# servos/SLAM

Measured on AMD Instinct MI355X. Metric: registered_scan_points_per_s, higher is better.
Workload: dtype f64 pose / f32 distance / int32 counts

## Files before the change

### slam_amd/csrc/grid.hip

```cpp
#include <algorithm>
#include <cmath>
#include <cstdlib>
#include <cstring>
#include <memory>
#include <vector>

#include "device_mem.hpp"
#include "grid_cell.hpp"

using namespace slam;

namespace {

struct GridView {
    int      sx, sy;
    int      ox, oy;
    double   res;
    double   max_range;
    double   pose_x, pose_y;
    int      rolling;
    int32_t *hits;
    int32_t *misses;
    unsigned long long *updates;
    int     *dirty;
    const int32_t *acc_hits, *acc_misses;
};

__device__ inline int storage_index(const GridView &g, int x, int y)
{
    int ix = x + g.ox, iy = y + g.oy;
    if (ix >= g.sx) ix -= g.sx;
    if (iy >= g.sy) iy -= g.sy;
    return ix + g.sx * iy;
}

__device__ inline bool point_cell(const GridView &g, float px, float py, int *cx, int *cy)
{
    return point_cell_of(g.sx, g.sy, g.res, g.max_range, g.pose_x, g.pose_y, g.rolling, px, py, cx, cy);
}

constexpr int kUpdateSlots = 1024;

__device__ inline void mark_dirty_rows(int *dirty, int row_lo, int row_hi )
{
    int lo = row_hi >= 0 ? row_lo : 0x7fffffff, nhi = row_hi >= 0 ? -row_hi : 0x7fffffff;
    for (int off = 32; off > 0; off >>= 1) {
        lo = min(lo, __shfl_xor(lo, off));
        nhi = min(nhi, __shfl_xor(nhi, off));
    }
    if ((threadIdx.x & 63) == 0 && lo != 0x7fffffff) {
        if (lo < __hip_atomic_load(&dirty[0], __ATOMIC_RELAXED, __HIP_MEMORY_SCOPE_AGENT)) atomicMin(&dirty[0], lo);
        if (nhi < __hip_atomic_load(&dirty[1], __ATOMIC_RELAXED, __HIP_MEMORY_SCOPE_AGENT)) atomicMin(&dirty[1], nhi);
    }
}

__device__ inline void block_add_updates(unsigned long long *slots, unsigned n)
{
    for (int off = 32; off > 0; off >>= 1) n += __shfl_xor((int)n, off);
    if ((threadIdx.x & 63) == 0 && n) {
        const unsigned wave = (blockIdx.x * (blockDim.x >> 6) + (threadIdx.x >> 6)) + blockIdx.y * 7919u;
        atomicAdd(&slots[wave & (kUpdateSlots - 1)], (unsigned long long)n);
    }
}

constexpr int kEndpointsPerBlock = 1024;

__global__ __launch_bounds__(256) void endpoints_kernel(GridView g, const float *obs, int n_obs,
                                                        const float *gnd, int n_gnd, int stride)
{
    __shared__ int      s_lo[4], s_nhi[4];
    __shared__ unsigned s_cnt[4];
    const int lane = threadIdx.x & 63, wave = threadIdx.x >> 6;
    int       lo = 0x7fffffff, nhi = 0x7fffffff;
    unsigned  cnt = 0;
#pragma unroll
    for (int k = 0; k < kEndpointsPerBlock / 256; ++k) {
        const int i = blockIdx.x * kEndpointsPerBlock + k * 256 + (int)threadIdx.x;
        bool      did = false;
        int       key = -1;
        if (i < n_obs + n_gnd) {
            const bool   is_obs = i < n_obs;
            const float *p = is_obs ? obs + (size_t)i * stride : gnd + (size_t)(i - n_obs) * stride;
            int cx, cy;
            if (point_cell(g, p[0], p[1], &cx, &cy)) {
                const int s = storage_index(g, cx, cy), row = s / g.sx;
                did = true;
                key = (is_obs ? 0 : g.sx * g.sy) + s;
                lo = min(lo, row);
                nhi = min(nhi, -row);
                ++cnt;
            }
        }
        const int                prev = __shfl_up(key, 1);
        const bool               head = did && (lane == 0 || prev != key);
        const unsigned long long heads = __ballot(head || !did);
        if (head) {
            const unsigned long long after = lane == 63 ? 0ull : heads >> (lane + 1);
            const int                len = after ? __builtin_ctzll(after) + 1 : 64 - lane;
            atomicAdd(&g.hits[key], len);
        }
    }
    for (int off = 32; off > 0; off >>= 1) {
        lo = min(lo, __shfl_xor(lo, off));
        nhi = min(nhi, __shfl_xor(nhi, off));
        cnt += (unsigned)__shfl_xor((int)cnt, off);
    }
    if (lane == 0) s_lo[wave] = lo, s_nhi[wave] = nhi, s_cnt[wave] = cnt;
    __syncthreads();
    if (threadIdx.x == 0) {
        lo = min(min(s_lo[0], s_lo[1]), min(s_lo[2], s_lo[3]));
        nhi = min(min(s_nhi[0], s_nhi[1]), min(s_nhi[2], s_nhi[3]));
        cnt = s_cnt[0] + s_cnt[1] + s_cnt[2] + s_cnt[3];
        if (lo != 0x7fffffff) {
            if (lo < __hip_atomic_load(&g.dirty[0], __ATOMIC_RELAXED, __HIP_MEMORY_SCOPE_AGENT)) atomicMin(&g.dirty[0], lo);
            if (nhi < __hip_atomic_load(&g.dirty[1], __ATOMIC_RELAXED, __HIP_MEMORY_SCOPE_AGENT)) atomicMin(&g.dirty[1], nhi);
        }
        if (cnt) atomicAdd(&g.updates[(blockIdx.x * 7u + blockIdx.y * 7919u) & (kUpdateSlots - 1)], (unsigned long long)cnt);
    }
}

struct Beam {
    short x0, y0, x1, y1;
};

constexpr int kTile = 128;
#ifndef SLAM_WALK_UNROLL
#define SLAM_WALK_UNROLL 4
#endif
constexpr int kWalkUnroll = SLAM_WALK_UNROLL;
#ifndef SLAM_WALK_STAGGER
#define SLAM_WALK_STAGGER 8
#endif
constexpr int kWalkStagger = SLAM_WALK_STAGGER;
constexpr int kTileStride = kTile + 1;
constexpr int kTileThreads = 1024;
constexpr int kChunk = 1024;
constexpr int kBlock = 64;

__device__ inline Beam make_beam(const GridView &g, float ox, float oy, float ex, float ey)
{
    Beam b;
    b.x0 = -1;
    b.y0 = b.x1 = b.y1 = 0;
    int x1, y1, x0, y0;
    if (!point_cell(g, ex, ey, &x1, &y1)) return b;
    if (!cell_coord(ox, g.res, g.sx / 2, &x0)) return b;
    if (!cell_coord(oy, g.res, g.sy / 2, &y0)) return b;
    if (x0 < 0 || y0 < 0 || x0 >= g.sx || y0 >= g.sy) return b;
    b.x0 = (short)x0;
    b.y0 = (short)y0;
    b.x1 = (short)x1;
    b.y1 = (short)y1;
    return b;
}

__device__ inline void store_beam_and_box(const Beam &b, bool in_range, int i, Beam *beams, int4 *block_box)
{
    if (in_range) beams[i] = b;
    const bool ok = in_range && b.x0 >= 0;
    int lo_x = ok ? min((int)b.x0, (int)b.x1) : 0x7fffffff, lo_y = ok ? min((int)b.y0, (int)b.y1) : 0x7fffffff;
    int hi_x = ok ? max((int)b.x0, (int)b.x1) : -1, hi_y = ok ? max((int)b.y0, (int)b.y1) : -1;
    for (int off = 32; off > 0; off >>= 1) {
        lo_x = min(lo_x, __shfl_xor(lo_x, off));
        lo_y = min(lo_y, __shfl_xor(lo_y, off));
        hi_x = max(hi_x, __shfl_xor(hi_x, off));
        hi_y = max(hi_y, __shfl_xor(hi_y, off));
    }
    if ((threadIdx.x & 63) == 0) block_box[i >> 6] = make_int4(lo_x, lo_y, hi_x, hi_y);
}

__global__ __launch_bounds__(kChunk) void beams_from_rays_kernel(GridView g, const float2 *origin,
                                                                 const float2 *end, int n, Beam *beams,
                                                                 int4 *block_box)
{
    const int  i = blockIdx.x * kChunk + threadIdx.x;
    const bool in = i < n;
    Beam       b;
    b.x0 = -1;
    b.y0 = b.x1 = b.y1 = 0;
    if (in) {
        const float2 o = origin[i], e = end[i];
        b = make_beam(g, o.x, o.y, e.x, e.y);
    }
    store_beam_and_box(b, in, i, beams, block_box);
}

__global__ __launch_bounds__(kChunk) void beams_from_scans_kernel(GridView g, const double2 *pts,
                                                                  const int *scan_off, int n_scans,
                                                                  const double *R, const double *t, int n,
                                                                  Beam *beams, int4 *block_box)
{
    const int  i = blockIdx.x * kChunk + threadIdx.x;
    const bool in = i < n;
    Beam       b;
    b.x0 = -1;
    b.y0 = b.x1 = b.y1 = 0;
    if (in) {
        int lo = (int)(((long long)i * n_scans) / max(n, 1));
        lo = min(max(lo, 0), n_scans - 1);
        int steps = 0;
        while (steps < 4 && scan_off[lo] > i) --lo, ++steps;
        while (steps < 4 && lo + 1 < n_scans && scan_off[lo + 1] <= i) ++lo, ++steps;
        if (scan_off[lo] > i || (lo + 1 < n_scans && scan_off[lo + 1] <= i)) {
            lo = 0;
            int hi = n_scans - 1;
            while (lo < hi) {
                const int mid = (lo + hi + 1) >> 1;
                if (scan_off[mid] <= i)
                    lo = mid;
                else
                    hi = mid - 1;
            }
        }
        const double *Rs = R + 4 * (size_t)lo, *ts = t + 2 * (size_t)lo;
        const double2 P = pts[i];
        const double cx = g.rolling ? g.pose_x : 0.0, cy = g.rolling ? g.pose_y : 0.0;
        const double gx = __dadd_rn(__dadd_rn(__dmul_rn(Rs[0], P.x), __dmul_rn(Rs[1], P.y)), ts[0]);
        const double gy = __dadd_rn(__dadd_rn(__dmul_rn(Rs[2], P.x), __dmul_rn(Rs[3], P.y)), ts[1]);
        const float  ex = (float)(g.rolling ? __dsub_rn(gx, cx) : gx), ey = (float)(g.rolling ? __dsub_rn(gy, cy) : gy);
        const float  ox = (float)(g.rolling ? __dsub_rn(ts[0], cx) : ts[0]);
        const float  oy = (float)(g.rolling ? __dsub_rn(ts[1], cy) : ts[1]);
        b = make_beam(g, ox, oy, ex, ey);
    }
    store_beam_and_box(b, in, i, beams, block_box);
}

__global__ __launch_bounds__(256) void raycast_global_kernel(GridView g, const Beam *beams, int n)
{
    const int i = blockIdx.x * 256 + threadIdx.x;
    unsigned  did = 0;
    int       rlo = 0, rhi = -1;
    if (i < n) {
        const Beam b = beams[i];
        if (b.x0 >= 0) {
            const int dx = abs(b.x1 - b.x0), dy = abs(b.y1 - b.y0);
            const int sx = b.x1 > b.x0 ? 1 : -1, sy = b.y1 > b.y0 ? 1 : -1;
            int x = b.x0, y = b.y0;
            if (dx >= dy) {
                int e = dx;
                for (int k = 0; k < dx; ++k) {
                    atomicAdd(&g.misses[storage_index(g, x, y)], 1);
                    x += sx;
                    e += 2 * dy;
                    if (e >= 2 * dx) {
                        y += sy;
                        e -= 2 * dx;
                    }
                }
                did = dx + 1;
            } else {
                int e = dy;
                for (int k = 0; k < dy; ++k) {
                    atomicAdd(&g.misses[storage_index(g, x, y)], 1);
                    y += sy;
                    e += 2 * dx;
                    if (e >= 2 * dy) {
                        x += sx;
                        e -= 2 * dy;
                    }
                }
                did = dy + 1;
            }
            atomicAdd(&g.hits[storage_index(g, b.x1, b.y1)], 1);
            const int ra = storage_index(g, 0, b.y0) / g.sx, rb = storage_index(g, 0, b.y1) / g.sx;
            const bool wraps = (ra <= rb) != (b.y0 <= b.y1);
            rlo = wraps ? 0 : min(ra, rb);
            rhi = wraps ? g.sy - 1 : max(ra, rb);
        }
    }
    mark_dirty_rows(g.dirty, rlo, rhi);
    block_add_updates(g.updates, did);
}


__device__ inline bool box_overlaps_tile(const int4 cb, int tx0, int ty0, int tx1, int ty1)
{
    return cb.z >= tx0 && cb.x <= tx1 && cb.w >= ty0 && cb.y <= ty1;
}

constexpr int kMaxLdsTiles = 2048;

template <int FILL>
__global__ __launch_bounds__(256) void tile_items_kernel(const int4 *block_box, int n_blocks, int tiles_x,
                                                         int n_tiles, int sx, int sy, int *cnt,
                                                         const int *item_off, int *items)
{
    const int t = (blockIdx.x * 256 + threadIdx.x) >> 6, lane = threadIdx.x & 63;
    if (t >= n_tiles) return;
    const int tx0 = (t % tiles_x) * kTile, ty0 = (t / tiles_x) * kTile;
    const int tx1 = min(tx0 + kTile, sx) - 1, ty1 = min(ty0 + kTile, sy) - 1;
    int       c = 0;
    const int base_out = FILL == 1 ? item_off[t] : 0;
    for (int base = 0; base < n_blocks; base += 256) {
        int4 cb[4];
#pragma unroll
        for (int j = 0; j < 4; ++j) {
            const int ch = base + 64 * j + lane;
            cb[j] = ch < n_blocks ? block_box[ch] : make_int4(0, 0, -1, -1);
        }
#pragma unroll
        for (int j = 0; j < 4; ++j) {
            const bool               ov = box_overlaps_tile(cb[j], tx0, ty0, tx1, ty1);
            const unsigned long long m = __ballot(ov);
            if (FILL && ov) items[base_out + c + __popcll(m & ((1ull << lane) - 1ull))] = base + 64 * j + lane;
            c += __popcll(m);
        }
    }
    if (FILL != 1 && lane == 0) cnt[t] = c;
}

__global__ __launch_bounds__(1024) void tile_items_wg_kernel(const int4 *block_box, int n_blocks, int tiles_x, int sx,
                                                             int sy, int *cnt, int *items, int *cursor)
{
    __shared__ int s_cnt[4][16], s_base;
    const int t = blockIdx.x, tid = threadIdx.x, lane = tid & 63, wave = tid >> 6;
    if (tid == 0) {
        s_base = 0;
        cursor[t] = 0;
        if (t == 0) cursor[gridDim.x] = 0;
    }
    const int tx0 = (t % tiles_x) * kTile, ty0 = (t / tiles_x) * kTile;
    const int tx1 = min(tx0 + kTile, sx) - 1, ty1 = min(ty0 + kTile, sy) - 1;
    const int base_out = t * n_blocks;
    for (int base = 0; base < n_blocks; base += 4096) {
        int4 cb[4];
#pragma unroll
        for (int j = 0; j < 4; ++j) {
            const int ch = base + 1024 * j + tid;
            cb[j] = ch < n_blocks ? block_box[ch] : make_int4(0, 0, -1, -1);
        }
        unsigned long long m[4];
#pragma unroll
        for (int j = 0; j < 4; ++j) {
            m[j] = __ballot(box_overlaps_tile(cb[j], tx0, ty0, tx1, ty1));
            if (lane == 0) s_cnt[j][wave] = __popcll(m[j]);
        }
        __syncthreads();
        int total = 0;
#pragma unroll
        for (int j = 0; j < 4; ++j)
            for (int w = 0; w < 16; ++w) {
                const int c = s_cnt[j][w];
                total += c;
            }
        int run = s_base;
#pragma unroll
        for (int j = 0; j < 4; ++j) {
            int mine = run;
            for (int w = 0; w < 16; ++w) {
                const int c = s_cnt[j][w];
                mine += w < wave ? c : 0;
                run += c;
            }
            if ((m[j] >> lane) & 1ull)
                items[base_out + mine + __popcll(m[j] & ((1ull << lane) - 1ull))] = base + 1024 * j + tid;
        }
        __syncthreads();
        if (tid == 0) s_base += total;
    }
    __syncthreads();
    if (tid == 0) cnt[t] = s_base;
}

__global__ __launch_bounds__(1024) void tile_scan_kernel(const int *cnt, int n_tiles, int *item_off, int *cursor)
{
    __shared__ int carry;
    __shared__ int wsum[16];
    const int tid = threadIdx.x;
    if (tid == 0) carry = 0;
    __syncthreads();
    for (int base = 0; base < n_tiles; base += 1024) {
        const int i = base + tid;
        const int v0 = i < n_tiles ? cnt[i] : 0;
        int       x0 = v0;
        for (int off = 1; off < 64; off <<= 1) {
            const int y0 = __shfl_up(x0, off);
            if ((tid & 63) >= off) x0 += y0;
        }
        if ((tid & 63) == 63) wsum[tid >> 6] = x0;
        __syncthreads();
        int w0 = 0;
        for (int w = 0; w < (tid >> 6); ++w) w0 += wsum[w];
        const int in0 = carry + w0 + x0;
        if (i < n_tiles) {
            item_off[i] = in0 - v0;
            cursor[i] = 0;
        }
        __syncthreads();
        if (tid == 1023) carry = in0;
        __syncthreads();
    }
    if (tid == 0) {
        item_off[n_tiles] = carry;
        cursor[n_tiles] = 0;
    }
}

__device__ inline int floor_div_small(int num, int den, float rden)
{
    const float qf = (float)num * rden;
    if (qf >= 65536.0f) return 65536;
    int       q = (int)qf;
    const int r = (int)((unsigned)num - (unsigned)__mul24(q, den));
    q += (r >= den) - (r < 0);
    return q;
}

constexpr int kChunkMin = 8;
constexpr int kChunkDefault = 16;
constexpr int kMaxAccBlocks = 1023;

template <bool MERGE>
__global__ __launch_bounds__(kTileThreads, 8) void raycast_tiled_kernel(GridView g, const Beam *beams, int n,
                                                                        const int *items, const int *item_off,
                                                                        int n_tiles, int *cursor, int tiles_x, int chunk,
                                                                        int ablate_arg, const int *cnt, int item_stride)
{
#ifdef SLAM_MEASURE
    const int ablate = ablate_arg;
#else
    constexpr int ablate = 0;
    (void)ablate_arg;
#endif
    __shared__ __attribute__((aligned(16))) unsigned tile[kTile * kTileStride];
    __shared__ int s_ticket, s_done, s_end;
    __shared__ unsigned long long s_desc[kMaxAccBlocks / kChunkMin];
    __shared__ int s_off[kMaxLdsTiles + 1], s_wsum[kTileThreads / 64], s_carry;
    __shared__ unsigned long long s_best[kTileThreads / 64];

    const int tid = threadIdx.x, lane = tid & 63;
    const bool in_lds = item_off == nullptr;
    if (in_lds) {
        if (tid == 0) s_carry = 0;
        __syncthreads();
        for (int base = 0; base < n_tiles; base += kTileThreads) {
            const int i = base + tid;
            const int v = i < n_tiles ? cnt[i] : 0;
            int       x = v;
            for (int off = 1; off < 64; off <<= 1) {
                const int y = __shfl_up(x, off);
                if (lane >= off) x += y;
            }
            if (lane == 63) s_wsum[tid >> 6] = x;
            __syncthreads();
            int w = 0;
            for (int k = 0; k < (tid >> 6); ++k) w += s_wsum[k];
            const int incl = s_carry + w + x;
            if (i < n_tiles) s_off[i] = incl - v;
            __syncthreads();
            if (tid == kTileThreads - 1) s_carry = incl;
            __syncthreads();
        }
        if (tid == 0) s_off[n_tiles] = s_carry;
        __syncthreads();
    }
    const auto list_start = [&](int t) { return in_lds ? s_off[t] : item_off[t]; };
    const int  total = list_start(n_tiles);
    unsigned   did = 0;
    int        d_lo = 0x7fffffff, d_hi = -1;
    if (total <= 0 || (ablate & 8)) {
        mark_dirty_rows(g.dirty, d_lo, d_hi);
        block_add_updates(g.updates, did);
        return;
    }
    int cur;
    {
        const int pos = (int)(((long long)blockIdx.x * total) / gridDim.x);
        int       lo = 0, hi = n_tiles - 1;
        while (lo < hi) {
            const int mid = (lo + hi + 1) >> 1;
            if (list_start(mid) <= pos)
                lo = mid;
            else
                hi = mid - 1;
        }
        cur = lo;
    }
    for (int i = tid * 4; i < kTile * kTileStride; i += kTileThreads * 4)
        *reinterpret_cast<uint4 *>(&tile[i]) = make_uint4(0u, 0u, 0u, 0u);

    const auto flush = [&](int t) {
        const int tx0 = (t % tiles_x) * kTile, ty0 = (t / tiles_x) * kTile;
        for (int i = (ablate & 2) ? kTile * kTile : tid; i < kTile * kTile; i += kTileThreads) {
            const int      lx = i & (kTile - 1), ly = i / kTile;
            const unsigned v = tile[ly * kTileStride + lx];
            if (!v) continue;
            tile[ly * kTileStride + lx] = 0u;
            const int s = storage_index(g, tx0 + lx, ty0 + ly);
            if (ablate & 128) {
                atomicAdd(reinterpret_cast<unsigned long long *>(g.hits) + s, ((unsigned long long)(v >> 16) << 32) | (v & 0xffffu));
            } else {
                if (v & 0xffffu) atomicAdd(&g.misses[s], (int)(v & 0xffffu));
                if (v >> 16) atomicAdd(&g.hits[s], (int)(v >> 16));
            }
            int row = ty0 + ly + g.oy;
            row -= row >= g.sy ? g.sy : 0;
            d_lo = min(d_lo, row);
            d_hi = max(d_hi, row);
        }
        if (tid == 0) atomicAdd(&cursor[n_tiles], 1);
    };

    const int  kMaxChunks = kMaxAccBlocks / chunk;
    const auto publish = [&](int c, int base, int np) {
        __hip_atomic_store(&s_desc[c], (1ull << 48) | ((unsigned long long)(unsigned)np << 32) | (unsigned)base, __ATOMIC_RELAXED,
                           __HIP_MEMORY_SCOPE_WORKGROUP);
        if (np < chunk) {
            atomicMin(&s_end, np > 0 ? c + 1 : c);
            s_done = 1;
        }
    };
    for (;;) {
        __syncthreads();
        for (int c = tid; c < kMaxChunks; c += kTileThreads) s_desc[c] = 0ull;
        if (tid == 0) {
            s_ticket = 0;
            s_done = 0;
            s_end = kMaxChunks;
        }
        __syncthreads();
        const int t = cur;
        if (tid == 0) {
            const int have_t = cnt[t];
            const int k = atomicAdd(&cursor[t], 2 * chunk);
            const int np0 = max(0, min(chunk, have_t - k));
            publish(0, k, np0);
            if (np0 == chunk) publish(1, k + chunk, max(0, min(chunk, have_t - k - chunk)));
        }
        const int tile_base = in_lds ? t * item_stride : item_off[t];
        const int tx0 = (t % tiles_x) * kTile, ty0 = (t / tiles_x) * kTile;
        const int tx1 = min(tx0 + kTile, g.sx) - 1, ty1 = min(ty0 + kTile, g.sy) - 1;

        int  fetch_c = -1, fetch_k = 0;
        auto settle = [&]() {
            if (fetch_c >= 0 && lane == 0) publish(fetch_c, fetch_k, max(0, min(chunk, cnt[t] - fetch_k)));
            fetch_c = -1;
        };
        auto wait_desc = [&](int c) -> unsigned long long {
            for (;;) {
                if (c >= __hip_atomic_load(&s_end, __ATOMIC_RELAXED, __HIP_MEMORY_SCOPE_WORKGROUP)) return 0ull;
                const unsigned long long d = __hip_atomic_load(&s_desc[c], __ATOMIC_RELAXED, __HIP_MEMORY_SCOPE_WORKGROUP);
                if (d != 0ull) return d;
                if (fetch_c >= 0)
                    settle();
                else
                    __builtin_amdgcn_s_sleep(1);
            }
        };
        auto grab = [&](int2 *raw) -> bool {
            int T = 0;
            if (lane == 0) T = atomicAdd(&s_ticket, 1);
            T = __builtin_amdgcn_readfirstlane(T);
            const int c = T / chunk, idx = T - c * chunk;
            if (c >= kMaxChunks) return false;
            const unsigned long long d = wait_desc(c);
            const int np = (int)((d >> 32) & 0xffffu), base = (int)(unsigned)(d & 0xffffffffull);
            if (idx >= np) return false;
            if (idx == 0 && np == chunk && c + 2 < kMaxChunks) {
                const unsigned long long d1 = wait_desc(c + 1);
                if ((int)((d1 >> 32) & 0xffffu) == chunk) {
                    settle();
                    if (lane == 0) fetch_k = atomicAdd(&cursor[t], chunk);
                    fetch_c = c + 2;
                }
            }
            const int bi = items[tile_base + base + idx] * kBlock + lane;
            *raw = bi < n ? *reinterpret_cast<const int2 *>(&beams[bi]) : make_int2(-1, 0);
            return true;
        };
        int2 raw = make_int2(-1, 0), raw_next = make_int2(-1, 0);
        bool have = grab(&raw);
        while (have) {
            const bool have_next = grab(&raw_next);

            int rem = 0, a = 0, e = 0, dv2 = 0, den = 1, step_u = 0, step_v = 0, to_end = 0;
            const int x0 = (short)(raw.x & 0xffff), y0 = raw.x >> 16;
            const int x1 = (short)(raw.y & 0xffff), y1 = raw.y >> 16;
            const bool maybe = x0 >= 0 && max(x0, x1) >= tx0 && min(x0, x1) <= tx1 && max(y0, y1) >= ty0 &&
                               min(y0, y1) <= ty1;
            if (__any(maybe) && !(ablate & 16)) {
                const int dx = abs(x1 - x0), dy = abs(y1 - y0);
                const bool xm = dx >= dy;
                const int  u0 = xm ? x0 : y0, v0 = xm ? y0 : x0, u1 = xm ? x1 : y1, v1 = xm ? y1 : x1;
                const int  du = xm ? dx : dy, dv = xm ? dy : dx;
                const int  tu0 = xm ? tx0 : ty0, tu1 = xm ? tx1 : ty1;
                const int  tv0 = xm ? ty0 : tx0, tv1 = xm ? ty1 : tx1;
                const bool up = u1 > u0, vp = v1 > v0;
                int        i_lo = max(0, up ? tu0 - u0 : u0 - tu1);
                int        i_hi = min(du, up ? tu1 - u0 : u0 - tu0);
                den = max(2 * du, 1);
                dv2 = 2 * dv;
                const float rden = __builtin_amdgcn_rcpf((float)den);
                const int k_lo = vp ? tv0 - v0 : v0 - tv1;
                const int k_hi = min(vp ? tv1 - v0 : v0 - tv0, dv);
                bool      enters = maybe && k_hi >= 0 && k_lo <= dv;
                if (enters && dv > 0 && !(ablate & 32)) {
                    const float rdv2 = __builtin_amdgcn_rcpf((float)dv2);
                    if (k_lo > 0) i_lo = max(i_lo, floor_div_small(__mul24(den, k_lo) - du + dv2 - 1, dv2, rdv2));
                    i_hi = min(i_hi, floor_div_small(__mul24(den, k_hi + 1) - du - 1, dv2, rdv2));
                }
                enters = enters && i_lo <= i_hi;
                if (enters && !(ablate & 64)) {
                    const int num = __mul24(i_lo, dv2) + du;
                    const int k = du ? floor_div_small(num, den, rden) : 0;
                    e = num - __mul24(k, den);
                    const int ul = (up ? u0 + i_lo : u0 - i_lo) - tu0, vl = (vp ? v0 + k : v0 - k) - tv0;
                    a = xm ? vl * kTileStride + ul : ul * kTileStride + vl;
                    step_u = (up ? 1 : -1) * (xm ? 1 : kTileStride);
                    step_v = (vp ? 1 : -1) * (xm ? kTileStride : 1);
                    rem = i_hi - i_lo + 1;
                    to_end = du - i_lo;
                    did += (unsigned)rem;
                }
            }
            if (ablate & 1) rem = 0;
            const bool hit_here = rem > 0 && to_end < rem;
            if (hit_here) atomicAdd(&tile[(y1 - ty0) * kTileStride + (x1 - tx0)], 0x10000u);
            int            miss = rem - (hit_here ? 1 : 0);
            unsigned char *tb = reinterpret_cast<unsigned char *>(tile);
            int            a4 = a * 4;
            const int      su4 = step_u * 4, sv4 = step_v * 4;
            const unsigned bias = 0u - (unsigned)den, udv2 = (unsigned)dv2;
            unsigned       eu = (unsigned)e + bias;
            const auto     advance = [&]() {
                const unsigned e2 = eu + udv2;
                const bool     carry = e2 < eu;
                a4 += su4 + (carry ? sv4 : 0);
                eu = e2 + (carry ? bias : 0u);
            };
            const auto add_miss = [&]() {
                if (!MERGE) {
                    atomicAdd(reinterpret_cast<unsigned *>(tb + a4), 1u);
                    return;
                }
                const int  prev = __builtin_amdgcn_update_dpp(-1, a4, 0x138 , 0xf, 0xf, false);
                const bool leader = a4 != prev;
                const unsigned long long on = __ballot(true), lead = __ballot(leader);
                if (lead == on) {
                    atomicAdd(reinterpret_cast<unsigned *>(tb + a4), 1u);
                } else {
                    const unsigned long long ends = lead | ~on;
                    const unsigned long long rest = lane == 63 ? 0ull : ends >> (lane + 1);
                    const unsigned run = rest ? (unsigned)__builtin_ctzll(rest) + 1u : (unsigned)(64 - lane);
                    if (leader) atomicAdd(reinterpret_cast<unsigned *>(tb + a4), run);
                }
            };
#pragma unroll
            for (int k = 0; k < kWalkStagger - 1; ++k) {
                if (lane % kWalkStagger > k && miss > 0) {
                    add_miss();
                    advance();
                    --miss;
                }
            }
            while (__any(miss >= kWalkUnroll)) {
                if (miss >= kWalkUnroll) {
#pragma unroll
                    for (int k = 0; k < kWalkUnroll; ++k) {
                        add_miss();
                        advance();
                    }
                    miss -= kWalkUnroll;
                }
            }
#pragma unroll
            for (int k = 0; k < kWalkUnroll - 1; ++k) {
                if (miss > k) add_miss();
                advance();
            }
            settle();
            have = have_next;
            raw = raw_next;
        }
        settle();
        __syncthreads();
        flush(t);
        if (s_done == 0) continue;
        unsigned long long best = 0ull;
        for (int u = tid; u < n_tiles; u += kTileThreads) {
            const int have_u = cnt[u];
            const int taken = __hip_atomic_load(&cursor[u], __ATOMIC_RELAXED, __HIP_MEMORY_SCOPE_AGENT);
            const int left = have_u - min(have_u, taken);
            const unsigned long long key = ((unsigned long long)(unsigned)left << 32) | (unsigned)u;
            best = left > 0 && key > best ? key : best;
        }
        for (int off = 32; off > 0; off >>= 1) {
            const unsigned long long o = __shfl_xor(best, off);
            best = o > best ? o : best;
        }
        if (lane == 0) s_best[tid >> 6] = best;
        __syncthreads();
        best = 0ull;
        for (int w = 0; w < kTileThreads / 64; ++w) best = s_best[w] > best ? s_best[w] : best;
        if (best == 0ull) break;
        cur = (int)(unsigned)(best & 0xffffffffull);
    }
    mark_dirty_rows(g.dirty, d_lo, d_hi);
    block_add_updates(g.updates, did);
}

__device__ inline bool row_in(const int *r, int row) { return row >= r[0] && row <= -r[1]; }

constexpr int kRangeBlocks = 1024;

__global__ __launch_bounds__(256) void reset_rows_kernel(int32_t *planes, size_t cells, int sx, int sy, const int *ranges)
{
    const int lo = max(ranges[0], 0), hi = min(-ranges[1], sy - 1);
    if (hi < lo) return;
    const int  per_row = (sx + 1023) / 1024;
    const long items = (long)(hi - lo + 1) * per_row;
    for (long it = blockIdx.x; it < items; it += gridDim.x) {
        const int row = lo + (int)(it / per_row), x = ((int)(it % per_row) * 256 + threadIdx.x) * 4;
        for (int k = 0; k < 4; ++k)
            if (x + k < sx) {
                planes[(size_t)row * sx + x + k] = 0;
                planes[cells + (size_t)row * sx + x + k] = 0;
            }
    }
}

__global__ void ranges_retire_kernel(int *ranges)
{
    if (threadIdx.x || blockIdx.x) return;
    ranges[2] = min(ranges[2], ranges[0]);
    ranges[3] = min(ranges[3], ranges[1]);
    ranges[0] = ranges[1] = 0x7f7f7f7f;
}

__global__ void ranges_fold_kernel(int *ranges, int lo, int hi)
{
    if (threadIdx.x || blockIdx.x) return;
    ranges[2] = min(min(ranges[2], ranges[0]), lo);
    ranges[3] = min(min(ranges[3], ranges[1]), -hi);
    if (ranges[0] >= lo && -ranges[1] <= hi) ranges[0] = ranges[1] = 0x7f7f7f7f;
}

__global__ void ranges_set_kernel(int *ranges, int mode, int lo, int hi, int sy)
{
    if (threadIdx.x || blockIdx.x) return;
    if (mode == 0) {
        ranges[2] = ranges[3] = 0x7f7f7f7f;
    } else if (mode == 1) {
        ranges[2] = 0;
        ranges[3] = -(sy - 1);
    } else {
        ranges[0] = min(ranges[0], lo);
        ranges[1] = min(ranges[1], -hi);
    }
}

__device__ inline void cell_value(int h, int m, double inc, double dec, double minp, double &v, int8_t &o)
{
    v = inc * (double)h;
    o = -1;
    if (h > 0 && v > minp) o = 100;
    v = v - dec * (double)m;
    if (m > 0 && v < minp) o = 0;
}

__device__ inline void finalize_cell(const GridView &g, int x, int y, double inc, double dec, double minp, double *num_pts, int8_t *occ)
{
    const int s = storage_index(g, x, y);
    const int h = g.hits[s] + (g.acc_hits ? g.acc_hits[s] : 0), m = g.misses[s] + (g.acc_misses ? g.acc_misses[s] : 0);
    double    v;
    int8_t    o;
    cell_value(h, m, inc, dec, minp, v, o);
    num_pts[x + (size_t)g.sx * y] = v;
    occ[x + (size_t)g.sx * y] = o;
}

template <bool RESET>
__device__ inline void finalize_quad(const GridView &g, int srow, int ix0, int y, double inc, double dec, double minp, double *num_pts,
                                     int8_t *occ)
{
    const size_t s0 = (size_t)srow * g.sx + ix0;
    int4         h = *reinterpret_cast<const int4 *>(g.hits + s0), m = *reinterpret_cast<const int4 *>(g.misses + s0);
    const bool   any = (h.x | h.y | h.z | h.w | m.x | m.y | m.z | m.w) != 0;
    if (g.acc_hits) {
        const int4 ah = *reinterpret_cast<const int4 *>(g.acc_hits + s0), am = *reinterpret_cast<const int4 *>(g.acc_misses + s0);
        h.x += ah.x, h.y += ah.y, h.z += ah.z, h.w += ah.w;
        m.x += am.x, m.y += am.y, m.z += am.z, m.w += am.w;
    }
    double v[4];
    int8_t o[4];
    cell_value(h.x, m.x, inc, dec, minp, v[0], o[0]);
    cell_value(h.y, m.y, inc, dec, minp, v[1], o[1]);
    cell_value(h.z, m.z, inc, dec, minp, v[2], o[2]);
    cell_value(h.w, m.w, inc, dec, minp, v[3], o[3]);
    int x0 = ix0 - g.ox;
    x0 += x0 < 0 ? g.sx : 0;
    const size_t w0 = (size_t)x0 + (size_t)g.sx * y;
    *reinterpret_cast<double2 *>(num_pts + w0) = make_double2(v[0], v[1]);
    *reinterpret_cast<double2 *>(num_pts + w0 + 2) = make_double2(v[2], v[3]);
    *reinterpret_cast<unsigned *>(occ + w0) = (unsigned)(unsigned char)o[0] | ((unsigned)(unsigned char)o[1] << 8) |
                                               ((unsigned)(unsigned char)o[2] << 16) | ((unsigned)(unsigned char)o[3] << 24);
    if (RESET && any) {
        *reinterpret_cast<int4 *>(g.hits + s0) = make_int4(0, 0, 0, 0);
        *reinterpret_cast<int4 *>(g.misses + s0) = make_int4(0, 0, 0, 0);
    }
}

template <bool RESET>
__device__ inline void finalize_rows(const GridView &g, int lo, int hi, double inc, double dec, double minp, double *num_pts, int8_t *occ)
{
    const bool quads = (g.sx & 3) == 0 && (g.ox & 3) == 0;
    const int  per_thread = quads ? 4 : 1;
    const int  per_row = (g.sx + 256 * per_thread - 1) / (256 * per_thread);
    const long items = (long)(hi - lo + 1) * per_row;
    for (long it = blockIdx.x; it < items; it += gridDim.x) {
        const int srow = lo + (int)(it / per_row), ix = ((int)(it % per_row) * 256 + (int)threadIdx.x) * per_thread;
        if (ix >= g.sx) continue;
        int y = srow - g.oy;
        y += y < 0 ? g.sy : 0;
        if (quads) {
            finalize_quad<RESET>(g, srow, ix, y, inc, dec, minp, num_pts, occ);
        } else {
            finalize_cell(g, ix, y, inc, dec, minp, num_pts, occ);
            if (RESET) {
                const int s = storage_index(g, ix, y);
                if (g.hits[s]) g.hits[s] = 0;
                if (g.misses[s]) g.misses[s] = 0;
            }
        }
    }
}

__global__ __launch_bounds__(256) void finalize_kernel(GridView g, double inc, double dec, double minp,
                                                       double *num_pts, int8_t *occ)
{
    const int x = blockIdx.x * 256 + threadIdx.x, y = blockIdx.y;
    if (x >= g.sx) return;
    finalize_cell(g, x, y, inc, dec, minp, num_pts, occ);
}

__global__ __launch_bounds__(256) void finalize_rows_kernel(GridView g, double inc, double dec, double minp, double *num_pts,
                                                            int8_t *occ, const int *ranges)
{
    const int lo = max(min(ranges[0], ranges[2]), 0), hi = min(max(-ranges[1], -ranges[3]), g.sy - 1);
    if (hi < lo) return;
    finalize_rows<false>(g, lo, hi, inc, dec, minp, num_pts, occ);
}

__global__ __launch_bounds__(256) void finalize_reset_rows_kernel(GridView g, double inc, double dec, double minp, double *num_pts,
                                                                  int8_t *occ, const int *ranges, int *next)
{
    const int t_lo = ranges[0], t_nhi = ranges[1];
    const int lo = max(min(t_lo, ranges[2]), 0), hi = min(max(-t_nhi, -ranges[3]), g.sy - 1);
    if (blockIdx.x == 0 && threadIdx.x == 0) {
        next[0] = next[1] = 0x7f7f7f7f;
        next[2] = t_lo;
        next[3] = t_nhi;
    }
    if (hi < lo) return;
    finalize_rows<true>(g, lo, hi, inc, dec, minp, num_pts, occ);
}

__global__ __launch_bounds__(256) void gather_counts_kernel(GridView g, int32_t *hits_w, int32_t *misses_w)
{
    const int x = blockIdx.x * 256 + threadIdx.x, y = blockIdx.y;
    if (x >= g.sx) return;
    const int s = storage_index(g, x, y);
    hits_w[x + (size_t)g.sx * y] = g.hits[s] + (g.acc_hits ? g.acc_hits[s] : 0);
    misses_w[x + (size_t)g.sx * y] = g.misses[s] + (g.acc_misses ? g.acc_misses[s] : 0);
}

__global__ __launch_bounds__(256) void fold_rows_kernel(int32_t *planes, int32_t *acc, size_t cells, int sx, int row_lo, int n_rows)
{
    const size_t i = (size_t)blockIdx.x * 256 + threadIdx.x, n = (size_t)n_rows * sx;
    if (i >= n) return;
    const size_t k = (size_t)row_lo * sx + i;
    for (int p = 0; p < 2; ++p) {
        const size_t j = p * cells + k;
        const int    v = planes[j];
        if (v) {
            acc[j] += v;
            planes[j] = 0;
        }
    }
}

__global__ __launch_bounds__(256) void roll_clear_kernel(GridView g, int dx, int dy, double *num_pts,
                                                         int8_t *occ_state)
{
    const int x = blockIdx.x * 256 + threadIdx.x, y = blockIdx.y;
    if (x >= g.sx) return;
    if (x < -dx || x >= g.sx - dx || y < -dy || y >= g.sy - dy) {
        const int s = storage_index(g, x, y);
        g.hits[s] = 0;
        g.misses[s] = 0;
        if (g.acc_hits) {
            const_cast<int32_t *>(g.acc_hits)[s] = 0;
            const_cast<int32_t *>(g.acc_misses)[s] = 0;
        }
        num_pts[s] = 0.0;
        occ_state[s] = -1;
    }
}

__global__ __launch_bounds__(256) void inorder_count_kernel(GridView g, const float *obs, int n_obs,
                                                            const float *gnd, int n_gnd, int stride,
                                                            unsigned long long *delta, int *touched,
                                                            int *n_touched)
{
    const int i = blockIdx.x * 256 + threadIdx.x;
    if (i >= n_obs + n_gnd) return;
    const bool   is_obs = i < n_obs;
    const float *p = is_obs ? obs + (size_t)i * stride : gnd + (size_t)(i - n_obs) * stride;
    int cx, cy;
    if (!point_cell(g, p[0], p[1], &cx, &cy)) return;
    const int s = storage_index(g, cx, cy);
    const unsigned long long old = atomicAdd(&delta[s], is_obs ? (1ull << 32) : 1ull);
    atomicAdd(is_obs ? &g.hits[s] : &g.misses[s], 1);
    if (old == 0ull) {
        const int row = s / g.sx;
        if (row < __hip_atomic_load(&g.dirty[0], __ATOMIC_RELAXED, __HIP_MEMORY_SCOPE_AGENT)) atomicMin(&g.dirty[0], row);
        if (-row < __hip_atomic_load(&g.dirty[1], __ATOMIC_RELAXED, __HIP_MEMORY_SCOPE_AGENT)) atomicMin(&g.dirty[1], -row);
    }
    if (old == 0ull) {
        const int k = atomicAdd(n_touched, 1);
        touched[k] = s;
    }
}

__global__ __launch_bounds__(256) void inorder_apply_kernel(GridView g, double inc, double dec, double minp,
                                                            unsigned long long *delta, const int *touched,
                                                            const int *n_touched, double *num_pts,
                                                            int8_t *occ_state, unsigned long long *updates)
{
    const int i = blockIdx.x * 256 + threadIdx.x;
    unsigned  did = 0;
    if (i < *n_touched) {
        const int s = touched[i];
        const unsigned long long d = delta[s];
        delta[s] = 0ull;
        const int h = (int)(d >> 32), m = (int)(d & 0xffffffffull);
        {
            double v = num_pts[s];
            int8_t o = occ_state[s];
            for (int k = 0; k < h; ++k) v = __dadd_rn(v, inc);
            if (h > 0 && v > minp) o = 100;
            for (int k = 0; k < m; ++k) v = __dsub_rn(v, dec);
            if (m > 0 && v < minp) o = 0;
            num_pts[s] = v;
            occ_state[s] = o;
            did = (unsigned)(h + m);
        }
    }
    block_add_updates(updates, did);
}

__global__ __launch_bounds__(256) void window_from_storage_kernel(GridView g, const double *num_s,
                                                                  const int8_t *occ_s, double *num_w,
                                                                  int8_t *occ_w)
{
    const int x = blockIdx.x * 256 + threadIdx.x, y = blockIdx.y;
    if (x >= g.sx) return;
    const int s = storage_index(g, x, y);
    num_w[x + (size_t)g.sx * y] = num_s[s];
    occ_w[x + (size_t)g.sx * y] = occ_s[s];
}

}

struct slam_grid {
    slam_grid_params prm;
    GridView         gv;
    size_t           cells = 0;
    OwnedArray<int32_t> d_planes;
    OwnedArray<double>  d_num_w;
    OwnedArray<int8_t>  d_occ_w;
    OwnedArray<double>  d_num_s;
    OwnedArray<int8_t>  d_occ_s;
    OwnedArray<unsigned long long> d_delta;
    OwnedArray<int>     d_touched;
    OwnedArray<unsigned long long> d_updates;
    OwnedArray<int>     d_dirty;
    OwnedArray<int32_t> d_acc;
    OwnedArray<Beam>    d_beams;
    OwnedArray<int4>    d_chunk_box;
    OwnedArray<int>     d_tile_cnt;
    OwnedArray<int>     d_tile_fill;
    OwnedArray<int>     d_cursor;
    OwnedArray<int>     d_items;
    int              n_cu = 256;
    int              seg_items = 0;
    int              last_chunks = 0;
    int              ablate = 0;
    int              wg_per_cu = 0;
    bool             merge = false;
    DevMem           d_stage;
    bool             state_from_inorder = false;
    long             shift_x = 0, shift_y = 0;
};

namespace {

int reserve(DevMem &b, size_t bytes) { return b.reserve(bytes, std::max(b.cap + b.cap / 4, (size_t)4096)); }

int reserve_beams(slam_grid *g, size_t n)
{
    SLAM_TRY(reserve(g->d_beams, n * sizeof(Beam)));
    const size_t chunks = (n + kBlock - 1) / kBlock + kChunk / kBlock;
    SLAM_TRY(reserve(g->d_chunk_box, chunks * sizeof(int4)));
    if (g->prm.raycast_impl != SLAM_RAYCAST_GLOBAL) {
        const size_t n_tiles = (size_t)((g->gv.sx + kTile - 1) / kTile) * ((g->gv.sy + kTile - 1) / kTile);
        if (!g->d_tile_cnt) {
            OwnedArray<int> cnt, fill, cursor;
            SLAM_TRY(cnt.alloc(n_tiles * sizeof(int)));
            SLAM_TRY(fill.alloc((n_tiles + 1) * sizeof(int)));
            SLAM_TRY(cursor.alloc((n_tiles + 1) * sizeof(int)));
            g->d_tile_cnt = std::move(cnt), g->d_tile_fill = std::move(fill), g->d_cursor = std::move(cursor);
        }
        SLAM_TRY(reserve(g->d_items, (chunks * n_tiles) * sizeof(int)));
    }
    return SLAM_OK;
}

int raycast_wg_per_cu(const slam_grid *g, int n_tiles) { return g->wg_per_cu > 0 ? g->wg_per_cu : 2; }
int raycast_workgroups(const slam_grid *g, int n_tiles)
{
    const int all = raycast_wg_per_cu(g, n_tiles) * g->n_cu;
    return g->prm.raycast_max_workgroups > 0 ? std::min(all, g->prm.raycast_max_workgroups) : all;
}

int walk_beams(slam_grid *g, int n, hipStream_t st)
{
    const int n_chunks = (n + kBlock - 1) / kBlock;
    if (g->prm.raycast_impl != SLAM_RAYCAST_GLOBAL) {
        const int tiles_x = (g->gv.sx + kTile - 1) / kTile, tiles_y = (g->gv.sy + kTile - 1) / kTile;
        const int n_tiles = tiles_x * tiles_y;
        int       *item_off = g->d_tile_fill;
        const dim3 tgrid((n_tiles * 64 + 255) / 256);
        const int  chunk = g->seg_items > 0 ? g->seg_items : kChunkDefault;
        const dim3 rgrid(raycast_workgroups(g, n_tiles));
        g->last_chunks = n_chunks;
        if (n_tiles <= kMaxLdsTiles) {
            hipLaunchKernelGGL(tile_items_wg_kernel, dim3(n_tiles), dim3(1024), 0, st, g->d_chunk_box, n_chunks, tiles_x,
                               g->gv.sx, g->gv.sy, g->d_tile_cnt, g->d_items, g->d_cursor);
            hipLaunchKernelGGL(g->merge ? raycast_tiled_kernel<true> : raycast_tiled_kernel<false>, rgrid, dim3(kTileThreads), 0, st,
                               g->gv, g->d_beams, n, g->d_items, (const int *)nullptr, n_tiles, g->d_cursor, tiles_x, chunk, g->ablate,
                               g->d_tile_cnt, n_chunks);
        } else {
            hipLaunchKernelGGL((tile_items_kernel<0>), tgrid, dim3(256), 0, st, g->d_chunk_box, n_chunks, tiles_x,
                               n_tiles, g->gv.sx, g->gv.sy, g->d_tile_cnt, item_off, g->d_items);
            hipLaunchKernelGGL(tile_scan_kernel, dim3(1), dim3(1024), 0, st, g->d_tile_cnt, n_tiles, item_off, g->d_cursor);
            hipLaunchKernelGGL((tile_items_kernel<1>), tgrid, dim3(256), 0, st, g->d_chunk_box, n_chunks, tiles_x,
                               n_tiles, g->gv.sx, g->gv.sy, g->d_tile_cnt, item_off, g->d_items);
            hipLaunchKernelGGL(g->merge ? raycast_tiled_kernel<true> : raycast_tiled_kernel<false>, rgrid, dim3(kTileThreads), 0, st,
                               g->gv, g->d_beams, n, g->d_items, item_off, n_tiles, g->d_cursor, tiles_x, chunk, g->ablate,
                               g->d_tile_cnt, 0);
        }
    } else {
        hipLaunchKernelGGL(raycast_global_kernel, dim3((n + 255) / 256), dim3(256), 0, st, g->gv, g->d_beams, n);
    }
    SLAM_HIP(hipGetLastError());
    return SLAM_OK;
}

dim3 grid2d(const slam_grid *g) { return dim3((g->gv.sx + 255) / 256, g->gv.sy); }

}

extern "C" {

void slam_grid_default_params(slam_grid_params *p)
{
    if (!p) return;
    p->max_range = 75.0;
    p->occupancy_increment = 1.0;
    p->occupancy_decrement = 0.3;
    p->min_cluster_points = 10;
    p->rolling = 1;
    p->raycast_impl = SLAM_RAYCAST_TILED;
    p->raycast_seg_items = 0;
    p->raycast_wg_per_cu = 0;
    p->raycast_max_workgroups = 0;
}

int slam_grid_create(int size_x, int size_y, double resolution, const slam_grid_params *params,
                     slam_grid_t **out)
{
    SLAM_REQUIRE(out, SLAM_E_INVALID, "slam_grid_create: null out pointer");
    *out = nullptr;
    SLAM_REQUIRE(size_x > 0 && size_y > 0 && size_x <= 32767 && size_y <= 32767 && resolution > 0,
                 SLAM_E_INVALID, "slam_grid_create: size must be 1..32767 cells and resolution > 0");
    SLAM_TRY(require_device());
    slam_grid *g = new (std::nothrow) slam_grid();
    SLAM_REQUIRE(g, SLAM_E_NOMEM, "slam_grid_create: out of host memory");
    if (params)
        g->prm = *params;
    else
        slam_grid_default_params(&g->prm);
    g->cells = (size_t)size_x * size_y;
    {
        int dev = 0;
        hipDeviceProp_t prop;
        if (hipGetDevice(&dev) == hipSuccess && hipGetDeviceProperties(&prop, dev) == hipSuccess)
            g->n_cu = std::max(1, prop.multiProcessorCount);
    }
    g->seg_items = g->prm.raycast_seg_items > 0 ? std::min(std::max(g->prm.raycast_seg_items, kChunkMin), kMaxAccBlocks / 2) : 0;
    if (g->prm.raycast_wg_per_cu > 0) g->wg_per_cu = std::min(g->prm.raycast_wg_per_cu, 8);
    g->merge = g->prm.raycast_impl == SLAM_RAYCAST_TILED_MERGE;
#ifdef SLAM_MEASURE
    if (const char *e = getenv("SLAM_RAYCAST_MERGE")) g->merge = atoi(e) != 0;
    if (const char *e = getenv("SLAM_RAYCAST_SEG")) g->seg_items = std::min(std::max(kChunkMin, atoi(e)), kMaxAccBlocks / 2);
    if (const char *e = getenv("SLAM_RAYCAST_ABLATE")) g->ablate = atoi(e);
    if (const char *e = getenv("SLAM_RAYCAST_WGPCU")) g->wg_per_cu = std::max(1, atoi(e));
#endif
    std::unique_ptr<slam_grid> guard(g);
    SLAM_TRY(g->d_planes.alloc(2 * g->cells * sizeof(int32_t)));
    SLAM_TRY(g->d_num_w.alloc(g->cells * sizeof(double)));
    SLAM_TRY(g->d_occ_w.alloc(g->cells));
    SLAM_TRY(g->d_num_s.alloc(g->cells * sizeof(double)));
    SLAM_TRY(g->d_occ_s.alloc(g->cells));
    SLAM_TRY(g->d_updates.alloc(kUpdateSlots * sizeof(unsigned long long)));
    SLAM_TRY(g->d_dirty.alloc(8 * sizeof(int)));
    GridView &v = g->gv;
    v.sx = size_x;
    v.sy = size_y;
    v.ox = v.oy = 0;
    v.res = resolution;
    v.max_range = g->prm.max_range;
    v.pose_x = v.pose_y = 0.0;
    v.rolling = g->prm.rolling ? 1 : 0;
    v.hits = g->d_planes;
    v.misses = g->d_planes + g->cells;
    v.updates = g->d_updates;
    v.dirty = g->d_dirty;
    v.acc_hits = v.acc_misses = nullptr;
    SLAM_TRY(slam_grid_clear(g, nullptr));
    SLAM_HIP(hipStreamSynchronize(nullptr));
    *out = guard.release();
    return SLAM_OK;
}

void slam_grid_destroy(slam_grid_t *g) { delete g; }

int slam_grid_clear(slam_grid_t *g, slam_stream_t stream)
{
    SLAM_REQUIRE(g, SLAM_E_INVALID, "null handle");
    hipStream_t st = as_stream(stream);
    SLAM_HIP(hipMemsetAsync(g->d_planes, 0, 2 * g->cells * sizeof(int32_t), st));
    SLAM_HIP(hipMemsetAsync(g->d_num_w, 0, g->cells * sizeof(double), st));
    SLAM_HIP(hipMemsetAsync(g->d_num_s, 0, g->cells * sizeof(double), st));
    SLAM_HIP(hipMemsetAsync(g->d_occ_w, 0xff, g->cells, st));
    SLAM_HIP(hipMemsetAsync(g->d_occ_s, 0xff, g->cells, st));
    SLAM_HIP(hipMemsetAsync(g->d_updates, 0, kUpdateSlots * sizeof(unsigned long long), st));
    SLAM_HIP(hipMemsetAsync(g->d_dirty, 0x7f, 8 * sizeof(int), st));
    if (g->d_acc) SLAM_HIP(hipMemsetAsync(g->d_acc, 0, 2 * g->cells * sizeof(int32_t), st));
    g->state_from_inorder = false;
    return SLAM_OK;
}

int slam_grid_reset_counts(slam_grid_t *g, slam_stream_t stream)
{
    SLAM_REQUIRE(g, SLAM_E_INVALID, "null handle");
    hipStream_t st = as_stream(stream);
    hipLaunchKernelGGL(reset_rows_kernel, dim3(kRangeBlocks), dim3(256), 0, st, g->d_planes, g->cells, g->gv.sx, g->gv.sy, g->gv.dirty);
    hipLaunchKernelGGL(ranges_retire_kernel, dim3(1), dim3(64), 0, st, g->gv.dirty);
    SLAM_HIP(hipGetLastError());
    return SLAM_OK;
}

int slam_grid_enable_accumulator(slam_grid_t *g)
{
    SLAM_REQUIRE(g, SLAM_E_INVALID, "null handle");
    if (g->d_acc) return SLAM_OK;
    SLAM_TRY(g->d_acc.alloc(2 * g->cells * sizeof(int32_t)));
    SLAM_HIP(hipMemset(g->d_acc, 0, 2 * g->cells * sizeof(int32_t)));
    g->gv.acc_hits = g->d_acc;
    g->gv.acc_misses = g->d_acc + g->cells;
    return SLAM_OK;
}

int slam_grid_fold(slam_grid_t *g, int row_lo, int row_hi, slam_stream_t stream)
{
    SLAM_REQUIRE(g && g->d_acc, SLAM_E_INVALID, "slam_grid_fold: needs slam_grid_enable_accumulator");
    hipStream_t st = as_stream(stream);
    if (row_hi >= row_lo) {
        SLAM_REQUIRE(row_lo >= 0 && row_hi < g->gv.sy, SLAM_E_INVALID, "slam_grid_fold: rows %d..%d outside the grid", row_lo, row_hi);
        const size_t n = (size_t)(row_hi - row_lo + 1) * g->gv.sx;
        hipLaunchKernelGGL(fold_rows_kernel, dim3((unsigned)((n + 255) / 256)), dim3(256), 0, st, g->d_planes, g->d_acc, g->cells,
                           g->gv.sx, row_lo, row_hi - row_lo + 1);
        SLAM_HIP(hipGetLastError());
    }
    if (row_hi >= row_lo)
        hipLaunchKernelGGL(ranges_fold_kernel, dim3(1), dim3(64), 0, st, g->gv.dirty, row_lo, row_hi);
    else
        hipLaunchKernelGGL(ranges_retire_kernel, dim3(1), dim3(64), 0, st, g->gv.dirty);
    SLAM_HIP(hipGetLastError());
    return SLAM_OK;
}

int slam_grid_mark_rows(slam_grid_t *g, int row_lo, int row_hi, slam_stream_t stream)
{
    SLAM_REQUIRE(g, SLAM_E_INVALID, "null handle");
    if (row_hi < row_lo) return SLAM_OK;
    SLAM_REQUIRE(row_lo >= 0 && row_hi < g->gv.sy, SLAM_E_INVALID, "slam_grid_mark_rows: rows %d..%d outside the grid", row_lo, row_hi);
    hipLaunchKernelGGL(ranges_set_kernel, dim3(1), dim3(64), 0, as_stream(stream), g->gv.dirty, 2, row_lo, row_hi, g->gv.sy);
    SLAM_HIP(hipGetLastError());
    return SLAM_OK;
}

int slam_grid_dirty_rows_dev(slam_grid_t *g, int32_t **d_range)
{
    SLAM_REQUIRE(g && d_range, SLAM_E_INVALID, "slam_grid_dirty_rows_dev: bad arguments");
    *d_range = g->gv.dirty;
    return SLAM_OK;
}

int slam_grid_dirty_rows(slam_grid_t *g, int *row_lo, int *row_hi)
{
    SLAM_REQUIRE(g && row_lo && row_hi, SLAM_E_INVALID, "slam_grid_dirty_rows: bad arguments");
    int r[2];
    SLAM_HIP(hipMemcpy(r, g->gv.dirty, sizeof r, hipMemcpyDeviceToHost));
    *row_lo = r[0] > g->gv.sy ? 0 : r[0];
    *row_hi = r[0] > g->gv.sy ? -1 : -r[1];
    return SLAM_OK;
}

int slam_grid_set_min_cluster_points(slam_grid_t *g, int v)
{
    SLAM_REQUIRE(g, SLAM_E_INVALID, "null handle");
    g->prm.min_cluster_points = v;
    hipLaunchKernelGGL(ranges_set_kernel, dim3(1), dim3(64), 0, nullptr, g->gv.dirty, 1, 0, 0, g->gv.sy);
    SLAM_HIP(hipGetLastError());
    return SLAM_OK;
}

int slam_grid_set_max_range(slam_grid_t *g, double v)
{
    SLAM_REQUIRE(g, SLAM_E_INVALID, "null handle");
    g->prm.max_range = v;
    g->gv.max_range = v;
    return SLAM_OK;
}

int slam_grid_get_pose(slam_grid_t *g, double *x, double *y)
{
    SLAM_REQUIRE(g, SLAM_E_INVALID, "null handle");
    if (x) *x = g->gv.pose_x;
    if (y) *y = g->gv.pose_y;
    return SLAM_OK;
}

int slam_grid_set_pose(slam_grid_t *g, double x, double y, slam_stream_t stream)
{
    SLAM_REQUIRE(g, SLAM_E_INVALID, "null handle");
    GridView &v = g->gv;
    if (!v.rolling) {
        v.pose_x = x;
        v.pose_y = y;
        return SLAM_OK;
    }
    const double xdiff = x - v.pose_x, ydiff = y - v.pose_y;
    const int    dx = (int)std::round(xdiff / v.res), dy = (int)std::round(ydiff / v.res);
    if (dx == 0 && dy == 0) return SLAM_OK;
    auto wrap = [](int o, int d, int n) {
        long v2 = ((long)o + d) % n;
        if (v2 < 0) v2 += n;
        return (int)v2;
    };
    v.ox = wrap(v.ox, dx, v.sx);
    v.oy = wrap(v.oy, dy, v.sy);
    v.pose_x += dx * v.res;
    v.pose_y += dy * v.res;
    g->shift_x += dx;
    g->shift_y += dy;
    hipLaunchKernelGGL(roll_clear_kernel, grid2d(g), dim3(256), 0, as_stream(stream), v, dx, dy, g->d_num_s,
                       g->d_occ_s);
    hipLaunchKernelGGL(ranges_set_kernel, dim3(1), dim3(64), 0, as_stream(stream), g->gv.dirty, 1, 0, 0, v.sy);
    SLAM_HIP(hipGetLastError());
    return SLAM_OK;
}

int slam_grid_add_endpoints_dev(slam_grid_t *g, const float *d_obs, int n_obs, const float *d_gnd, int n_gnd,
                                int stride, slam_stream_t stream)
{
    SLAM_REQUIRE(g && n_obs >= 0 && n_gnd >= 0 && stride >= 2, SLAM_E_INVALID,
                 "slam_grid_add_endpoints_dev: bad arguments");
    const int n = n_obs + n_gnd;
    if (n == 0) return SLAM_OK;
    hipLaunchKernelGGL(endpoints_kernel, dim3((n + kEndpointsPerBlock - 1) / kEndpointsPerBlock), dim3(256), 0, as_stream(stream), g->gv, d_obs,
                       n_obs, d_gnd, n_gnd, stride);
    SLAM_HIP(hipGetLastError());
    return SLAM_OK;
}

static int stage_points(slam_grid *g, const float *obs, int n_obs, const float *gnd, int n_gnd, int stride,
                        float **d_obs, float **d_gnd)
{
    const size_t bo = (size_t)n_obs * stride * sizeof(float), bg = (size_t)n_gnd * stride * sizeof(float);
    SLAM_TRY(reserve(g->d_stage, bo + bg + 16));
    *d_obs = g->d_stage.as<float>();
    *d_gnd = *d_obs + (size_t)n_obs * stride;
    if (bo) SLAM_HIP(hipMemcpyAsync(*d_obs, obs, bo, hipMemcpyHostToDevice, nullptr));
    if (bg) SLAM_HIP(hipMemcpyAsync(*d_gnd, gnd, bg, hipMemcpyHostToDevice, nullptr));
    return SLAM_OK;
}

int slam_grid_add_endpoints(slam_grid_t *g, const float *obs, int n_obs, const float *gnd, int n_gnd,
                            int stride)
{
    SLAM_REQUIRE(g && n_obs >= 0 && n_gnd >= 0 && stride >= 2 && (obs || !n_obs) && (gnd || !n_gnd),
                 SLAM_E_INVALID, "slam_grid_add_endpoints: bad arguments");
    SLAM_TRY(require_device());
    float *d_obs, *d_gnd;
    SLAM_TRY(stage_points(g, obs, n_obs, gnd, n_gnd, stride, &d_obs, &d_gnd));
    SLAM_TRY(slam_grid_add_endpoints_dev(g, d_obs, n_obs, d_gnd, n_gnd, stride, nullptr));
    SLAM_HIP(hipStreamSynchronize(nullptr));
    return SLAM_OK;
}

int slam_grid_raycast_dev(slam_grid_t *g, const float *d_origin_xy, const float *d_end_xy, int n,
                          slam_stream_t stream)
{
    SLAM_REQUIRE(g && n >= 0 && (n == 0 || (d_origin_xy && d_end_xy)), SLAM_E_INVALID,
                 "slam_grid_raycast_dev: bad arguments");
    if (n == 0) return SLAM_OK;
    hipStream_t st = as_stream(stream);
    SLAM_TRY(reserve_beams(g, (size_t)n));
    const int n_chunks = (n + kChunk - 1) / kChunk;
    hipLaunchKernelGGL(beams_from_rays_kernel, dim3(n_chunks), dim3(kChunk), 0, st, g->gv,
                       reinterpret_cast<const float2 *>(d_origin_xy), reinterpret_cast<const float2 *>(d_end_xy),
                       n, g->d_beams, g->d_chunk_box);
    SLAM_HIP(hipGetLastError());
    return walk_beams(g, n, st);
}

int slam_grid_raycast(slam_grid_t *g, const float *origin_xy, const float *end_xy, int n)
{
    SLAM_REQUIRE(g && n >= 0 && (n == 0 || (origin_xy && end_xy)), SLAM_E_INVALID,
                 "slam_grid_raycast: bad arguments");
    SLAM_TRY(require_device());
    if (n == 0) return SLAM_OK;
    float *d_o, *d_e;
    SLAM_TRY(stage_points(g, origin_xy, n, end_xy, n, 2, &d_o, &d_e));
    SLAM_TRY(slam_grid_raycast_dev(g, d_o, d_e, n, nullptr));
    SLAM_HIP(hipStreamSynchronize(nullptr));
    return SLAM_OK;
}

int slam_grid_reserve(slam_grid_t *g, int max_beams)
{
    SLAM_REQUIRE(g && max_beams >= 0, SLAM_E_INVALID, "slam_grid_reserve: bad arguments");
    return max_beams ? reserve_beams(g, (size_t)max_beams) : SLAM_OK;
}

int slam_grid_raycast_scans_dev(slam_grid_t *g, const double *d_pts, const int32_t *d_scan_off, int n_scans,
                                int n_points, const double *d_R, const double *d_t, slam_stream_t stream)
{
    SLAM_REQUIRE(g && n_scans >= 0 && n_points >= 0 && d_scan_off && d_R && d_t, SLAM_E_INVALID,
                 "slam_grid_raycast_scans_dev: bad arguments");
    if (n_scans == 0 || n_points == 0) return SLAM_OK;
    hipStream_t st = as_stream(stream);
    const int   n = n_points;
    SLAM_TRY(reserve_beams(g, (size_t)n));
    const int n_chunks = (n + kChunk - 1) / kChunk;
    hipLaunchKernelGGL(beams_from_scans_kernel, dim3(n_chunks), dim3(kChunk), 0, st, g->gv,
                       reinterpret_cast<const double2 *>(d_pts), d_scan_off, n_scans, d_R, d_t, n, g->d_beams,
                       g->d_chunk_box);
    SLAM_HIP(hipGetLastError());
    return walk_beams(g, n, st);
}

int slam_grid_finalize(slam_grid_t *g, slam_stream_t stream)
{
    SLAM_REQUIRE(g, SLAM_E_INVALID, "null handle");
    if (g->state_from_inorder)
        hipLaunchKernelGGL(finalize_kernel, grid2d(g), dim3(256), 0, as_stream(stream), g->gv, g->prm.occupancy_increment,
                           g->prm.occupancy_decrement, (double)g->prm.min_cluster_points, g->d_num_w, g->d_occ_w);
    else
        hipLaunchKernelGGL(finalize_rows_kernel, dim3(kRangeBlocks), dim3(256), 0, as_stream(stream), g->gv, g->prm.occupancy_increment,
                           g->prm.occupancy_decrement, (double)g->prm.min_cluster_points, g->d_num_w, g->d_occ_w, g->gv.dirty);
    hipLaunchKernelGGL(ranges_set_kernel, dim3(1), dim3(64), 0, as_stream(stream), g->gv.dirty, 0, 0, 0, g->gv.sy);
    SLAM_HIP(hipGetLastError());
    g->state_from_inorder = false;
    return SLAM_OK;
}

int slam_grid_finalize_reset(slam_grid_t *g, slam_stream_t stream)
{
    SLAM_REQUIRE(g, SLAM_E_INVALID, "null handle");
    bool capturing = false;
    if (stream) {
        hipStreamCaptureStatus cap = hipStreamCaptureStatusNone;
        if (hipStreamIsCapturing(as_stream(stream), &cap) == hipSuccess)
            capturing = cap != hipStreamCaptureStatusNone;
        else
            (void)hipGetLastError();
    }
    if (g->state_from_inorder || capturing) {
        SLAM_TRY(slam_grid_finalize(g, stream));
        return slam_grid_reset_counts(g, stream);
    }
    int *cur = g->gv.dirty, *next = cur == g->d_dirty ? g->d_dirty + 4 : g->d_dirty;
    hipLaunchKernelGGL(finalize_reset_rows_kernel, dim3(kRangeBlocks), dim3(256), 0, as_stream(stream), g->gv, g->prm.occupancy_increment,
                       g->prm.occupancy_decrement, (double)g->prm.min_cluster_points, g->d_num_w, g->d_occ_w, cur, next);
    SLAM_HIP(hipGetLastError());
    g->gv.dirty = next;
    return SLAM_OK;
}

namespace {
struct CloudTransform {
    double r[9], t[3];
};
__global__ __launch_bounds__(256) void transform_cloud_kernel(const float *in, int n, int stride, CloudTransform T, float *out)
{
    const int i = blockIdx.x * 256 + threadIdx.x;
    if (i >= n) return;
    const double px = in[(size_t)i * stride], py = in[(size_t)i * stride + 1], pz = in[(size_t)i * stride + 2];
#pragma unroll
    for (int k = 0; k < 3; ++k)
        out[3 * (size_t)i + k] = (float)__dadd_rn(
            __dadd_rn(__dadd_rn(__dmul_rn(T.r[3 * k], px), __dmul_rn(T.r[3 * k + 1], py)), __dmul_rn(T.r[3 * k + 2], pz)), T.t[k]);
}
}

int slam_grid_transform_cloud_dev(const float *d_in_xyz, int n, int stride, const double R[9], const double t[3], float *d_out_xyz,
                                  slam_stream_t stream)
{
    SLAM_REQUIRE(n >= 0 && stride >= 3 && R && t && ((d_in_xyz && d_out_xyz) || n == 0), SLAM_E_INVALID,
                 "slam_grid_transform_cloud_dev: bad arguments");
    SLAM_TRY(require_device());
    if (n == 0) return SLAM_OK;
    CloudTransform T;
    for (int k = 0; k < 9; ++k) T.r[k] = R[k];
    for (int k = 0; k < 3; ++k) T.t[k] = t[k];
    hipLaunchKernelGGL(transform_cloud_kernel, dim3((n + 255) / 256), dim3(256), 0, as_stream(stream), d_in_xyz, n, stride, T, d_out_xyz);
    SLAM_HIP(hipGetLastError());
    return SLAM_OK;
}

int slam_grid_add_scan_inorder_dev(slam_grid_t *g, const float *d_obs, int n_obs, const float *d_gnd, int n_gnd, int stride,
                                   slam_stream_t stream)
{
    SLAM_REQUIRE(g && n_obs >= 0 && n_gnd >= 0 && stride >= 2 && (d_obs || !n_obs) && (d_gnd || !n_gnd), SLAM_E_INVALID,
                 "slam_grid_add_scan_inorder_dev: bad arguments");
    SLAM_TRY(require_device());
    const int n = n_obs + n_gnd;
    if (n == 0) return SLAM_OK;
    hipStream_t st = as_stream(stream);
    if (!g->d_delta) {
        SLAM_TRY(g->d_delta.alloc(g->cells * sizeof(unsigned long long)));
        SLAM_HIP(hipMemsetAsync(g->d_delta, 0, g->cells * sizeof(unsigned long long), st));
    }
    SLAM_TRY(reserve(g->d_touched, ((size_t)n + 1) * sizeof(int)));
    int *counter = g->d_touched + n;
    SLAM_HIP(hipMemsetAsync(counter, 0, sizeof(int), st));
    hipLaunchKernelGGL(inorder_count_kernel, dim3((n + 255) / 256), dim3(256), 0, st, g->gv, d_obs, n_obs, d_gnd, n_gnd, stride,
                       g->d_delta, g->d_touched, counter);
    hipLaunchKernelGGL(inorder_apply_kernel, dim3((n + 255) / 256), dim3(256), 0, st, g->gv, g->prm.occupancy_increment,
                       g->prm.occupancy_decrement, (double)g->prm.min_cluster_points, g->d_delta, g->d_touched, counter,
                       g->d_num_s, g->d_occ_s, g->d_updates);
    SLAM_HIP(hipGetLastError());
    g->state_from_inorder = true;
    return SLAM_OK;
}

int slam_grid_add_scan_inorder(slam_grid_t *g, const float *obs, int n_obs, const float *gnd, int n_gnd,
                               int stride)
{
    SLAM_REQUIRE(g && n_obs >= 0 && n_gnd >= 0 && stride >= 2 && (obs || !n_obs) && (gnd || !n_gnd),
                 SLAM_E_INVALID, "slam_grid_add_scan_inorder: bad arguments");
    SLAM_TRY(require_device());
    if (n_obs + n_gnd == 0) return SLAM_OK;
    float *d_obs, *d_gnd;
    SLAM_TRY(stage_points(g, obs, n_obs, gnd, n_gnd, stride, &d_obs, &d_gnd));
    SLAM_TRY(slam_grid_add_scan_inorder_dev(g, d_obs, n_obs, d_gnd, n_gnd, stride, nullptr));
    SLAM_HIP(hipStreamSynchronize(nullptr));
    return SLAM_OK;
}

int slam_grid_read_counts(slam_grid_t *g, int32_t *hits, int32_t *misses)
{
    SLAM_REQUIRE(g && hits && misses, SLAM_E_INVALID, "slam_grid_read_counts: bad arguments");
    SLAM_TRY(require_device());
    DevMem scratch;
    SLAM_TRY(scratch.alloc(2 * g->cells * sizeof(int32_t)));
    int32_t *tmp = scratch.as<int32_t>();
    hipLaunchKernelGGL(gather_counts_kernel, grid2d(g), dim3(256), 0, nullptr, g->gv, tmp, tmp + g->cells);
    SLAM_HIP(hipMemcpy(hits, tmp, g->cells * sizeof(int32_t), hipMemcpyDeviceToHost));
    SLAM_HIP(hipMemcpy(misses, tmp + g->cells, g->cells * sizeof(int32_t), hipMemcpyDeviceToHost));
    return SLAM_OK;
}

static int sync_window_state(slam_grid *g)
{
    if (g->state_from_inorder) {
        hipLaunchKernelGGL(window_from_storage_kernel, grid2d(g), dim3(256), 0, nullptr, g->gv, g->d_num_s,
                           g->d_occ_s, g->d_num_w, g->d_occ_w);
        SLAM_HIP(hipGetLastError());
    }
    return SLAM_OK;
}

int slam_grid_read_occupancy(slam_grid_t *g, int8_t *occ)
{
    SLAM_REQUIRE(g && occ, SLAM_E_INVALID, "slam_grid_read_occupancy: bad arguments");
    SLAM_TRY(require_device());
    SLAM_TRY(sync_window_state(g));
    SLAM_HIP(hipMemcpy(occ, g->d_occ_w, g->cells, hipMemcpyDeviceToHost));
    return SLAM_OK;
}

int slam_grid_read_num_pts(slam_grid_t *g, double *num_pts)
{
    SLAM_REQUIRE(g && num_pts, SLAM_E_INVALID, "slam_grid_read_num_pts: bad arguments");
    SLAM_TRY(require_device());
    SLAM_TRY(sync_window_state(g));
    SLAM_HIP(hipMemcpy(num_pts, g->d_num_w, g->cells * sizeof(double), hipMemcpyDeviceToHost));
    return SLAM_OK;
}

int slam_grid_total_updates(slam_grid_t *g, uint64_t *n)
{
    SLAM_REQUIRE(g && n, SLAM_E_INVALID, "slam_grid_total_updates: bad arguments");
    SLAM_TRY(require_device());
    std::vector<unsigned long long> v(kUpdateSlots, 0);
    SLAM_HIP(hipMemcpy(v.data(), g->d_updates, kUpdateSlots * sizeof(unsigned long long), hipMemcpyDeviceToHost));
    uint64_t sum = 0;
    for (unsigned long long x : v) sum += x;
    *n = sum;
    return SLAM_OK;
}

int slam_grid_info(slam_grid_t *g, int *size_x, int *size_y, double *resolution, int *origin_x, int *origin_y)
{
    SLAM_REQUIRE(g, SLAM_E_INVALID, "null handle");
    if (size_x) *size_x = g->gv.sx;
    if (size_y) *size_y = g->gv.sy;
    if (resolution) *resolution = g->gv.res;
    if (origin_x) *origin_x = g->gv.ox;
    if (origin_y) *origin_y = g->gv.oy;
    return SLAM_OK;
}

int slam_grid_window_cell(slam_grid_t *g, int *cell_x, int *cell_y)
{
    SLAM_REQUIRE(g, SLAM_E_INVALID, "null handle");
    if (cell_x) *cell_x = (int)g->shift_x;
    if (cell_y) *cell_y = (int)g->shift_y;
    return SLAM_OK;
}

int slam_grid_raycast_stats(slam_grid_t *g, int *n_tiles, int *n_items, int *n_segments)
{
    SLAM_REQUIRE(g, SLAM_E_INVALID, "null handle");
    const int tiles = ((g->gv.sx + kTile - 1) / kTile) * ((g->gv.sy + kTile - 1) / kTile);
    if (n_tiles) *n_tiles = tiles;
    if (n_items) *n_items = 0;
    if (n_segments) *n_segments = 0;
    if (!g->d_tile_fill) return SLAM_OK;
    SLAM_HIP(hipDeviceSynchronize());
    std::vector<int> cnt((size_t)tiles);
    SLAM_HIP(hipMemcpy(cnt.data(), g->d_tile_cnt, sizeof(int) * (size_t)tiles, hipMemcpyDeviceToHost));
    long items = 0;
    for (int c : cnt) items += c;
    if (n_items) *n_items = (int)items;
    if (n_segments) SLAM_HIP(hipMemcpy(n_segments, g->d_cursor + tiles, sizeof(int), hipMemcpyDeviceToHost));
    return SLAM_OK;
}

int slam_grid_counts_dev(slam_grid_t *g, int32_t **d_planes, size_t *n_ints)
{
    SLAM_REQUIRE(g && d_planes, SLAM_E_INVALID, "slam_grid_counts_dev: bad arguments");
    *d_planes = g->d_planes;
    if (n_ints) *n_ints = 2 * g->cells;
    return SLAM_OK;
}

}
```

Before: 1.032 billion.

## Track dirty column ranges and cull tile-beam pairs with angular sectors

Adds a column dirty range next to the row range so finalize and reset passes sweep only the touched column span, not full rows. Each 64-beam chunk now records a shared-origin angular sector, which tile binning uses to skip tiles outside the wedge even when the bounding box overlaps. Dirty-row marking moves out of the raycast kernels into the binning kernels (or a small box-join kernel) using the chunk boxes. This cuts per-cell finalize work and raycast tile items, at the cost of extra shuffles, sector storage and a doubled dirty buffer layout.

Result: no change. 1.035 billion (median of 6 runs) (+0.3%).

```diff
diff --git a/slam_amd/csrc/grid.hip b/slam_amd/csrc/grid.hip
--- a/slam_amd/csrc/grid.hip
+++ b/slam_amd/csrc/grid.hip
@@ -41,17 +41,10 @@
 
 constexpr int kUpdateSlots = 1024;
 
-__device__ inline void mark_dirty_rows(int *dirty, int row_lo, int row_hi )
-{
-    int lo = row_hi >= 0 ? row_lo : 0x7fffffff, nhi = row_hi >= 0 ? -row_hi : 0x7fffffff;
-    for (int off = 32; off > 0; off >>= 1) {
-        lo = min(lo, __shfl_xor(lo, off));
-        nhi = min(nhi, __shfl_xor(nhi, off));
-    }
-    if ((threadIdx.x & 63) == 0 && lo != 0x7fffffff) {
-        if (lo < __hip_atomic_load(&dirty[0], __ATOMIC_RELAXED, __HIP_MEMORY_SCOPE_AGENT)) atomicMin(&dirty[0], lo);
-        if (nhi < __hip_atomic_load(&dirty[1], __ATOMIC_RELAXED, __HIP_MEMORY_SCOPE_AGENT)) atomicMin(&dirty[1], nhi);
-    }
+__device__ inline void widen_range(int *range, int lo, int nhi)
+{
+    if (lo < __hip_atomic_load(&range[0], __ATOMIC_RELAXED, __HIP_MEMORY_SCOPE_AGENT)) atomicMin(&range[0], lo);
+    if (nhi < __hip_atomic_load(&range[1], __ATOMIC_RELAXED, __HIP_MEMORY_SCOPE_AGENT)) atomicMin(&range[1], nhi);
 }
 
 __device__ inline void block_add_updates(unsigned long long *slots, unsigned n)
@@ -68,10 +61,11 @@
 __global__ __launch_bounds__(256) void endpoints_kernel(GridView g, const float *obs, int n_obs,
                                                         const float *gnd, int n_gnd, int stride)
 {
-    __shared__ int      s_lo[4], s_nhi[4];
+    __shared__ int      s_lo[4], s_nhi[4], s_clo[4], s_cnhi[4];
     __shared__ unsigned s_cnt[4];
     const int lane = threadIdx.x & 63, wave = threadIdx.x >> 6;
     int       lo = 0x7fffffff, nhi = 0x7fffffff;
+    int       clo = 0x7fffffff, cnhi = 0x7fffffff;
     unsigned  cnt = 0;
 #pragma unroll
     for (int k = 0; k < kEndpointsPerBlock / 256; ++k) {
@@ -88,6 +82,8 @@
                 key = (is_obs ? 0 : g.sx * g.sy) + s;
                 lo = min(lo, row);
                 nhi = min(nhi, -row);
+                clo = min(clo, s - row * g.sx);
+                cnhi = min(cnhi, row * g.sx - s);
                 ++cnt;
             }
         }
@@ -103,17 +99,21 @@
     for (int off = 32; off > 0; off >>= 1) {
         lo = min(lo, __shfl_xor(lo, off));
         nhi = min(nhi, __shfl_xor(nhi, off));
+        clo = min(clo, __shfl_xor(clo, off));
+        cnhi = min(cnhi, __shfl_xor(cnhi, off));
         cnt += (unsigned)__shfl_xor((int)cnt, off);
     }
-    if (lane == 0) s_lo[wave] = lo, s_nhi[wave] = nhi, s_cnt[wave] = cnt;
+    if (lane == 0) s_lo[wave] = lo, s_nhi[wave] = nhi, s_clo[wave] = clo, s_cnhi[wave] = cnhi, s_cnt[wave] = cnt;
     __syncthreads();
     if (threadIdx.x == 0) {
         lo = min(min(s_lo[0], s_lo[1]), min(s_lo[2], s_lo[3]));
         nhi = min(min(s_nhi[0], s_nhi[1]), min(s_nhi[2], s_nhi[3]));
+        clo = min(min(s_clo[0], s_clo[1]), min(s_clo[2], s_clo[3]));
+        cnhi = min(min(s_cnhi[0], s_cnhi[1]), min(s_cnhi[2], s_cnhi[3]));
         cnt = s_cnt[0] + s_cnt[1] + s_cnt[2] + s_cnt[3];
         if (lo != 0x7fffffff) {
-            if (lo < __hip_atomic_load(&g.dirty[0], __ATOMIC_RELAXED, __HIP_MEMORY_SCOPE_AGENT)) atomicMin(&g.dirty[0], lo);
-            if (nhi < __hip_atomic_load(&g.dirty[1], __ATOMIC_RELAXED, __HIP_MEMORY_SCOPE_AGENT)) atomicMin(&g.dirty[1], nhi);
+            widen_range(g.dirty, lo, nhi);
+            widen_range(g.dirty + 4, clo, cnhi);
         }
         if (cnt) atomicAdd(&g.updates[(blockIdx.x * 7u + blockIdx.y * 7919u) & (kUpdateSlots - 1)], (unsigned long long)cnt);
     }
@@ -154,24 +154,46 @@
     return b;
 }
 
-__device__ inline void store_beam_and_box(const Beam &b, bool in_range, int i, Beam *beams, int4 *block_box)
+__device__ inline long long cross2(int ax, int ay, int bx, int by) { return (long long)ax * by - (long long)ay * bx; }
+
+__device__ inline void store_beam_and_box(const Beam &b, bool in_range, int i, Beam *beams, int4 *block_box, int4 *block_sector)
 {
     if (in_range) beams[i] = b;
     const bool ok = in_range && b.x0 >= 0;
     int lo_x = ok ? min((int)b.x0, (int)b.x1) : 0x7fffffff, lo_y = ok ? min((int)b.y0, (int)b.y1) : 0x7fffffff;
     int hi_x = ok ? max((int)b.x0, (int)b.x1) : -1, hi_y = ok ? max((int)b.y0, (int)b.y1) : -1;
+    const int dx = ok ? b.x1 - b.x0 : 0, dy = ok ? b.y1 - b.y0 : 0;
+    int       lx = dx, ly = dy, rx = dx, ry = dy;
     for (int off = 32; off > 0; off >>= 1) {
         lo_x = min(lo_x, __shfl_xor(lo_x, off));
         lo_y = min(lo_y, __shfl_xor(lo_y, off));
         hi_x = max(hi_x, __shfl_xor(hi_x, off));
         hi_y = max(hi_y, __shfl_xor(hi_y, off));
-    }
-    if ((threadIdx.x & 63) == 0) block_box[i >> 6] = make_int4(lo_x, lo_y, hi_x, hi_y);
+        const int  blx = __shfl_xor(lx, off), bly = __shfl_xor(ly, off), brx = __shfl_xor(rx, off), bry = __shfl_xor(ry, off);
+        const bool tl = (lx | ly) == 0 || cross2(lx, ly, blx, bly) < 0;
+        const bool tr = (rx | ry) == 0 || cross2(rx, ry, brx, bry) > 0;
+        lx = tl ? blx : lx, ly = tl ? bly : ly;
+        rx = tr ? brx : rx, ry = tr ? bry : ry;
+    }
+    lx = __builtin_amdgcn_readfirstlane(lx), ly = __builtin_amdgcn_readfirstlane(ly);
+    rx = __builtin_amdgcn_readfirstlane(rx), ry = __builtin_amdgcn_readfirstlane(ry);
+    const unsigned long long have = __ballot(ok);
+    const int                first = have ? __builtin_ctzll(have) : 0;
+    const int                ox = __shfl((int)b.x0, first), oy = __shfl((int)b.y0, first);
+    const long long          cl = cross2(lx, ly, dx, dy), cr = cross2(dx, dy, rx, ry);
+    const bool against = (cl == 0 && (long long)lx * dx + (long long)ly * dy < 0) || (cr == 0 && (long long)rx * dx + (long long)ry * dy < 0);
+    const bool bad = ok && (b.x0 != ox || b.y0 != oy || cl < 0 || cr < 0 || against);
+    const bool valid = have != 0ull && __ballot(bad) == 0ull && cross2(lx, ly, rx, ry) >= 0;
+    if ((threadIdx.x & 63) == 0) {
+        block_box[i >> 6] = make_int4(lo_x, lo_y, hi_x, hi_y);
+        const auto pack = [](int lo, int hi) { return (int)(((unsigned)lo & 0xffffu) | ((unsigned)hi << 16)); };
+        block_sector[i >> 6] = make_int4(pack(ox, oy), pack(lx, ly), pack(rx, ry), valid ? 1 : 0);
+    }
 }
 
 __global__ __launch_bounds__(kChunk) void beams_from_rays_kernel(GridView g, const float2 *origin,
                                                                  const float2 *end, int n, Beam *beams,
-                                                                 int4 *block_box)
+                                                                 int4 *block_box, int4 *block_sector)
 {
     const int  i = blockIdx.x * kChunk + threadIdx.x;
     const bool in = i < n;
@@ -182,13 +204,13 @@
         const float2 o = origin[i], e = end[i];
         b = make_beam(g, o.x, o.y, e.x, e.y);
     }
-    store_beam_and_box(b, in, i, beams, block_box);
+    store_beam_and_box(b, in, i, beams, block_box, block_sector);
 }
 
 __global__ __launch_bounds__(kChunk) void beams_from_scans_kernel(GridView g, const double2 *pts,
                                                                   const int *scan_off, int n_scans,
                                                                   const double *R, const double *t, int n,
-                                                                  Beam *beams, int4 *block_box)
+                                                                  Beam *beams, int4 *block_box, int4 *block_sector)
 {
     const int  i = blockIdx.x * kChunk + threadIdx.x;
     const bool in = i < n;
@@ -222,14 +244,13 @@
         const float  oy = (float)(g.rolling ? __dsub_rn(ts[1], cy) : ts[1]);
         b = make_beam(g, ox, oy, ex, ey);
     }
-    store_beam_and_box(b, in, i, beams, block_box);
+    store_beam_and_box(b, in, i, beams, block_box, block_sector);
 }
 
 __global__ __launch_bounds__(256) void raycast_global_kernel(GridView g, const Beam *beams, int n)
 {
     const int i = blockIdx.x * 256 + threadIdx.x;
     unsigned  did = 0;
-    int       rlo = 0, rhi = -1;
     if (i < n) {
         const Beam b = beams[i];
         if (b.x0 >= 0) {
@@ -262,31 +283,91 @@
                 did = dy + 1;
             }
             atomicAdd(&g.hits[storage_index(g, b.x1, b.y1)], 1);
-            const int ra = storage_index(g, 0, b.y0) / g.sx, rb = storage_index(g, 0, b.y1) / g.sx;
-            const bool wraps = (ra <= rb) != (b.y0 <= b.y1);
-            rlo = wraps ? 0 : min(ra, rb);
-            rhi = wraps ? g.sy - 1 : max(ra, rb);
-        }
-    }
-    mark_dirty_rows(g.dirty, rlo, rhi);
+        }
+    }
     block_add_updates(g.updates, did);
 }
 
 
+struct BoxMark {
+    int *dirty;
+    int  sx, sy, ox, oy;
+};
+
+__device__ inline void box_join(int4 &u, const int4 cb)
+{
+    u.x = min(u.x, cb.x), u.y = min(u.y, cb.y), u.z = max(u.z, cb.z), u.w = max(u.w, cb.w);
+}
+
+__device__ inline int4 box_wave_join(int4 u)
+{
+    for (int off = 32; off > 0; off >>= 1) {
+        u.x = min(u.x, __shfl_xor(u.x, off)), u.y = min(u.y, __shfl_xor(u.y, off));
+        u.z = max(u.z, __shfl_xor(u.z, off)), u.w = max(u.w, __shfl_xor(u.w, off));
+    }
+    return u;
+}
+
+__device__ inline void mark_window_box(const BoxMark &k, const int4 u)
+{
+    if (u.z < 0) return;
+    int ra = u.y + k.oy, rb = u.w + k.oy, ca = u.x + k.ox, cb = u.z + k.ox;
+    ra -= ra >= k.sy ? k.sy : 0, rb -= rb >= k.sy ? k.sy : 0;
+    ca -= ca >= k.sx ? k.sx : 0, cb -= cb >= k.sx ? k.sx : 0;
+    if (ra > rb) ra = 0, rb = k.sy - 1;
+    if (ca > cb) ca = 0, cb = k.sx - 1;
+    widen_range(k.dirty, ra, -rb);
+    widen_range(k.dirty + 4, ca, -cb);
+}
+
+constexpr int4 kEmptyBox = {0x7fffffff, 0x7fffffff, -1, -1};
+
+__global__ __launch_bounds__(1024) void mark_boxes_kernel(const int4 *block_box, int n_blocks, BoxMark mark)
+{
+    __shared__ int4 s_u[16];
+    int4            u = kEmptyBox;
+    for (int ch = threadIdx.x; ch < n_blocks; ch += 1024) box_join(u, block_box[ch]);
+    u = box_wave_join(u);
+    if ((threadIdx.x & 63) == 0) s_u[threadIdx.x >> 6] = u;
+    __syncthreads();
+    if (threadIdx.x == 0) {
+        for (int w = 1; w < 16; ++w) box_join(u, s_u[w]);
+        mark_window_box(mark, u);
+    }
+}
+
 __device__ inline bool box_overlaps_tile(const int4 cb, int tx0, int ty0, int tx1, int ty1)
 {
     return cb.z >= tx0 && cb.x <= tx1 && cb.w >= ty0 && cb.y <= ty1;
 }
 
+__device__ inline bool sector_misses_tile(const int4 s, int tx0, int ty0, int tx1, int ty1)
+{
+    if (!s.w) return false;
+    const int ox = (short)(s.x & 0xffff), oy = s.x >> 16;
+    const int lx = (short)(s.y & 0xffff), ly = s.y >> 16, rx = (short)(s.z & 0xffff), ry = s.z >> 16;
+    const int ax = tx0 - 1 - ox, bx = tx1 + 1 - ox, ay = ty0 - 1 - oy, by = ty1 + 1 - oy;
+    const bool beyond_l = cross2(lx, ly, ax, ay) < 0 && cross2(lx, ly, bx, ay) < 0 && cross2(lx, ly, ax, by) < 0 && cross2(lx, ly, bx, by) < 0;
+    const bool beyond_r = cross2(ax, ay, rx, ry) < 0 && cross2(bx, ay, rx, ry) < 0 && cross2(ax, by, rx, ry) < 0 && cross2(bx, by, rx, ry) < 0;
+    return beyond_l || beyond_r;
+}
+
+__device__ inline bool block_in_tile(const int4 cb, const int4 *block_sector, int ch, int tx0, int ty0, int tx1, int ty1)
+{
+    if (!box_overlaps_tile(cb, tx0, ty0, tx1, ty1)) return false;
+    return !sector_misses_tile(block_sector[ch], tx0, ty0, tx1, ty1);
+}
+
 constexpr int kMaxLdsTiles = 2048;
 
 template <int FILL>
-__global__ __launch_bounds__(256) void tile_items_kernel(const int4 *block_box, int n_blocks, int tiles_x,
+__global__ __launch_bounds__(256) void tile_items_kernel(const int4 *block_box, const int4 *block_sector, int n_blocks, int tiles_x,
                                                          int n_tiles, int sx, int sy, int *cnt,
-                                                         const int *item_off, int *items)
+                                                         const int *item_off, int *items, BoxMark mark)
 {
     const int t = (blockIdx.x * 256 + threadIdx.x) >> 6, lane = threadIdx.x & 63;
     if (t >= n_tiles) return;
+    int4 u = kEmptyBox;
     const int tx0 = (t % tiles_x) * kTile, ty0 = (t / tiles_x) * kTile;
     const int tx1 = min(tx0 + kTile, sx) - 1, ty1 = min(ty0 + kTile, sy) - 1;
     int       c = 0;
@@ -297,22 +378,29 @@
         for (int j = 0; j < 4; ++j) {
             const int ch = base + 64 * j + lane;
             cb[j] = ch < n_blocks ? block_box[ch] : make_int4(0, 0, -1, -1);
+            if (FILL == 0 && t == 0 && ch < n_blocks) box_join(u, cb[j]);
         }
 #pragma unroll
         for (int j = 0; j < 4; ++j) {
-            const bool               ov = box_overlaps_tile(cb[j], tx0, ty0, tx1, ty1);
+            const bool               ov = block_in_tile(cb[j], block_sector, base + 64 * j + lane, tx0, ty0, tx1, ty1);
             const unsigned long long m = __ballot(ov);
             if (FILL && ov) items[base_out + c + __popcll(m & ((1ull << lane) - 1ull))] = base + 64 * j + lane;
             c += __popcll(m);
         }
     }
     if (FILL != 1 && lane == 0) cnt[t] = c;
-}
-
-__global__ __launch_bounds__(1024) void tile_items_wg_kernel(const int4 *block_box, int n_blocks, int tiles_x, int sx,
-                                                             int sy, int *cnt, int *items, int *cursor)
-{
-    __shared__ int s_cnt[4][16], s_base;
+    if (FILL == 0 && t == 0) {
+        u = box_wave_join(u);
+        if (lane == 0) mark_window_box(mark, u);
+    }
+}
+
+__global__ __launch_bounds__(1024) void tile_items_wg_kernel(const int4 *block_box, const int4 *block_sector, int n_blocks, int tiles_x, int sx,
+                                                             int sy, int *cnt, int *items, int *cursor, BoxMark mark)
+{
+    __shared__ int  s_cnt[4][16], s_base;
+    __shared__ int4 s_u[16];
+    int4            u = kEmptyBox;
     const int t = blockIdx.x, tid = threadIdx.x, lane = tid & 63, wave = tid >> 6;
     if (tid == 0) {
         s_base = 0;
@@ -328,11 +416,12 @@
         for (int j = 0; j < 4; ++j) {
             const int ch = base + 1024 * j + tid;
             cb[j] = ch < n_blocks ? block_box[ch] : make_int4(0, 0, -1, -1);
+            if (t == 0 && ch < n_blocks) box_join(u, cb[j]);
         }
         unsigned long long m[4];
 #pragma unroll
         for (int j = 0; j < 4; ++j) {
-            m[j] = __ballot(box_overlaps_tile(cb[j], tx0, ty0, tx1, ty1));
+            m[j] = __ballot(block_in_tile(cb[j], block_sector, base + 1024 * j + tid, tx0, ty0, tx1, ty1));
             if (lane == 0) s_cnt[j][wave] = __popcll(m[j]);
         }
         __syncthreads();
@@ -358,8 +447,18 @@
         __syncthreads();
         if (tid == 0) s_base += total;
     }
+    if (t == 0) {
+        u = box_wave_join(u);
+        if (lane == 0) s_u[wave] = u;
+    }
     __syncthreads();
-    if (tid == 0) cnt[t] = s_base;
+    if (tid == 0) {
+        cnt[t] = s_base;
+        if (t == 0) {
+            for (int w = 1; w < 16; ++w) box_join(u, s_u[w]);
+            mark_window_box(mark, u);
+        }
+    }
 }
 
 __global__ __launch_bounds__(1024) void tile_scan_kernel(const int *cnt, int n_tiles, int *item_off, int *cursor)
@@ -457,9 +556,7 @@
     const auto list_start = [&](int t) { return in_lds ? s_off[t] : item_off[t]; };
     const int  total = list_start(n_tiles);
     unsigned   did = 0;
-    int        d_lo = 0x7fffffff, d_hi = -1;
     if (total <= 0 || (ablate & 8)) {
-        mark_dirty_rows(g.dirty, d_lo, d_hi);
         block_add_updates(g.updates, did);
         return;
     }
@@ -493,10 +590,6 @@
                 if (v & 0xffffu) atomicAdd(&g.misses[s], (int)(v & 0xffffu));
                 if (v >> 16) atomicAdd(&g.hits[s], (int)(v >> 16));
             }
-            int row = ty0 + ly + g.oy;
-            row -= row >= g.sy ? g.sy : 0;
-            d_lo = min(d_lo, row);
-            d_hi = max(d_hi, row);
         }
         if (tid == 0) atomicAdd(&cursor[n_tiles], 1);
     };
@@ -695,11 +788,21 @@
         if (best == 0ull) break;
         cur = (int)(unsigned)(best & 0xffffffffull);
     }
-    mark_dirty_rows(g.dirty, d_lo, d_hi);
     block_add_updates(g.updates, did);
 }
 
 __device__ inline bool row_in(const int *r, int row) { return row >= r[0] && row <= -r[1]; }
+
+constexpr int kNoRange = 0x7f7f7f7f;
+
+__device__ inline void column_hull(const int *a, const int *b, int sx, int align, int *c_lo, int *c_hi)
+{
+    int lo = b ? min(a[0], b[0]) : a[0], hi = b ? max(-a[1], -b[1]) : -a[1];
+    if (lo > hi) lo = 0, hi = sx - 1;
+    lo = max(lo, 0), hi = min(hi, sx - 1);
+    *c_lo = lo / align * align;
+    *c_hi = min(hi / align * align + align - 1, sx - 1);
+}
 
 constexpr int kRangeBlocks = 1024;
 
@@ -707,12 +810,14 @@
 {
     const int lo = max(ranges[0], 0), hi = min(-ranges[1], sy - 1);
     if (hi < lo) return;
-    const int  per_row = (sx + 1023) / 1024;
+    int c_lo, c_hi;
+    column_hull(ranges + 4, nullptr, sx, 1, &c_lo, &c_hi);
+    const int  per_row = (c_hi - c_lo + 1 + 1023) / 1024;
     const long items = (long)(hi - lo + 1) * per_row;
     for (long it = blockIdx.x; it < items; it += gridDim.x) {
-        const int row = lo + (int)(it / per_row), x = ((int)(it % per_row) * 256 + threadIdx.x) * 4;
+        const int row = lo + (int)(it / per_row), x = c_lo + ((int)(it % per_row) * 256 + threadIdx.x) * 4;
         for (int k = 0; k < 4; ++k)
-            if (x + k < sx) {
+            if (x + k <= c_hi) {
                 planes[(size_t)row * sx + x + k] = 0;
                 planes[cells + (size_t)row * sx + x + k] = 0;
             }
@@ -724,28 +829,36 @@
     if (threadIdx.x || blockIdx.x) return;
     ranges[2] = min(ranges[2], ranges[0]);
     ranges[3] = min(ranges[3], ranges[1]);
-    ranges[0] = ranges[1] = 0x7f7f7f7f;
-}
-
-__global__ void ranges_fold_kernel(int *ranges, int lo, int hi)
+    ranges[6] = min(ranges[6], ranges[4]);
+    ranges[7] = min(ranges[7], ranges[5]);
+    ranges[0] = ranges[1] = ranges[4] = ranges[5] = kNoRange;
+}
+
+__global__ void ranges_fold_kernel(int *ranges, int lo, int hi, int sx)
 {
     if (threadIdx.x || blockIdx.x) return;
     ranges[2] = min(min(ranges[2], ranges[0]), lo);
     ranges[3] = min(min(ranges[3], ranges[1]), -hi);
-    if (ranges[0] >= lo && -ranges[1] <= hi) ranges[0] = ranges[1] = 0x7f7f7f7f;
-}
-
-__global__ void ranges_set_kernel(int *ranges, int mode, int lo, int hi, int sy)
+    ranges[6] = 0;
+    ranges[7] = -(sx - 1);
+    if (ranges[0] >= lo && -ranges[1] <= hi) ranges[0] = ranges[1] = ranges[4] = ranges[5] = kNoRange;
+}
+
+__global__ void ranges_set_kernel(int *ranges, int mode, int lo, int hi, int sx, int sy)
 {
     if (threadIdx.x || blockIdx.x) return;
     if (mode == 0) {
-        ranges[2] = ranges[3] = 0x7f7f7f7f;
+        ranges[2] = ranges[3] = ranges[6] = ranges[7] = kNoRange;
     } else if (mode == 1) {
         ranges[2] = 0;
         ranges[3] = -(sy - 1);
+        ranges[6] = 0;
+        ranges[7] = -(sx - 1);
     } else {
         ranges[0] = min(ranges[0], lo);
         ranges[1] = min(ranges[1], -hi);
+        ranges[4] = 0;
+        ranges[5] = -(sx - 1);
     }
 }
 
@@ -801,23 +914,28 @@
 }
 
 template <bool RESET>
-__device__ inline void finalize_rows(const GridView &g, int lo, int hi, double inc, double dec, double minp, double *num_pts, int8_t *occ)
+__device__ inline void finalize_rows(const GridView &g, int lo, int hi, const int *cols_a, const int *cols_b, double inc, double dec,
+                                     double minp, double *num_pts, int8_t *occ)
 {
     const bool quads = (g.sx & 3) == 0 && (g.ox & 3) == 0;
     const int  per_thread = quads ? 4 : 1;
-    const int  per_row = (g.sx + 256 * per_thread - 1) / (256 * per_thread);
+    int        c_lo, c_hi;
+    column_hull(cols_a, cols_b, g.sx, per_thread, &c_lo, &c_hi);
+    const int  per_row = (c_hi - c_lo + 1 + 256 * per_thread - 1) / (256 * per_thread);
     const long items = (long)(hi - lo + 1) * per_row;
     for (long it = blockIdx.x; it < items; it += gridDim.x) {
-        const int srow = lo + (int)(it / per_row), ix = ((int)(it % per_row) * 256 + (int)threadIdx.x) * per_thread;
-        if (ix >= g.sx) continue;
+        const int srow = lo + (int)(it / per_row), ix = c_lo + ((int)(it % per_row) * 256 + (int)threadIdx.x) * per_thread;
+        if (ix > c_hi) continue;
         int y = srow - g.oy;
         y += y < 0 ? g.sy : 0;
         if (quads) {
             finalize_quad<RESET>(g, srow, ix, y, inc, dec, minp, num_pts, occ);
         } else {
-            finalize_cell(g, ix, y, inc, dec, minp, num_pts, occ);
+            int x = ix - g.ox;
+            x += x < 0 ? g.sx : 0;
+            finalize_cell(g, x, y, inc, dec, minp, num_pts, occ);
             if (RESET) {
-                const int s = storage_index(g, ix, y);
+                const size_t s = (size_t)srow * g.sx + ix;
                 if (g.hits[s]) g.hits[s] = 0;
                 if (g.misses[s]) g.misses[s] = 0;
             }
@@ -838,7 +956,7 @@
 {
     const int lo = max(min(ranges[0], ranges[2]), 0), hi = min(max(-ranges[1], -ranges[3]), g.sy - 1);
     if (hi < lo) return;
-    finalize_rows<false>(g, lo, hi, inc, dec, minp, num_pts, occ);
+    finalize_rows<false>(g, lo, hi, ranges + 4, ranges + 6, inc, dec, minp, num_pts, occ);
 }
 
 __global__ __launch_bounds__(256) void finalize_reset_rows_kernel(GridView g, double inc, double dec, double minp, double *num_pts,
@@ -847,12 +965,14 @@
     const int t_lo = ranges[0], t_nhi = ranges[1];
     const int lo = max(min(t_lo, ranges[2]), 0), hi = min(max(-t_nhi, -ranges[3]), g.sy - 1);
     if (blockIdx.x == 0 && threadIdx.x == 0) {
-        next[0] = next[1] = 0x7f7f7f7f;
+        next[0] = next[1] = next[4] = next[5] = kNoRange;
         next[2] = t_lo;
         next[3] = t_nhi;
+        next[6] = ranges[4];
+        next[7] = ranges[5];
     }
     if (hi < lo) return;
-    finalize_rows<true>(g, lo, hi, inc, dec, minp, num_pts, occ);
+    finalize_rows<true>(g, lo, hi, ranges + 4, ranges + 6, inc, dec, minp, num_pts, occ);
 }
 
 __global__ __launch_bounds__(256) void gather_counts_kernel(GridView g, int32_t *hits_w, int32_t *misses_w)
@@ -912,9 +1032,9 @@
     const unsigned long long old = atomicAdd(&delta[s], is_obs ? (1ull << 32) : 1ull);
     atomicAdd(is_obs ? &g.hits[s] : &g.misses[s], 1);
     if (old == 0ull) {
-        const int row = s / g.sx;
-        if (row < __hip_atomic_load(&g.dirty[0], __ATOMIC_RELAXED, __HIP_MEMORY_SCOPE_AGENT)) atomicMin(&g.dirty[0], row);
-        if (-row < __hip_atomic_load(&g.dirty[1], __ATOMIC_RELAXED, __HIP_MEMORY_SCOPE_AGENT)) atomicMin(&g.dirty[1], -row);
+        const int row = s / g.sx, col = s - row * g.sx;
+        widen_range(g.dirty, row, -row);
+        widen_range(g.dirty + 4, col, -col);
     }
     if (old == 0ull) {
         const int k = atomicAdd(n_touched, 1);
@@ -978,6 +1098,7 @@
     OwnedArray<int32_t> d_acc;
     OwnedArray<Beam>    d_beams;
     OwnedArray<int4>    d_chunk_box;
+    OwnedArray<int4>    d_chunk_sector;
     OwnedArray<int>     d_tile_cnt;
     OwnedArray<int>     d_tile_fill;
     OwnedArray<int>     d_cursor;
@@ -1002,6 +1123,7 @@
     SLAM_TRY(reserve(g->d_beams, n * sizeof(Beam)));
     const size_t chunks = (n + kBlock - 1) / kBlock + kChunk / kBlock;
     SLAM_TRY(reserve(g->d_chunk_box, chunks * sizeof(int4)));
+    SLAM_TRY(reserve(g->d_chunk_sector, chunks * sizeof(int4)));
     if (g->prm.raycast_impl != SLAM_RAYCAST_GLOBAL) {
         const size_t n_tiles = (size_t)((g->gv.sx + kTile - 1) / kTile) * ((g->gv.sy + kTile - 1) / kTile);
         if (!g->d_tile_cnt) {
@@ -1034,23 +1156,26 @@
         const int  chunk = g->seg_items > 0 ? g->seg_items : kChunkDefault;
         const dim3 rgrid(raycast_workgroups(g, n_tiles));
         g->last_chunks = n_chunks;
+        const BoxMark mark = {g->gv.dirty, g->gv.sx, g->gv.sy, g->gv.ox, g->gv.oy};
         if (n_tiles <= kMaxLdsTiles) {
-            hipLaunchKernelGGL(tile_items_wg_kernel, dim3(n_tiles), dim3(1024), 0, st, g->d_chunk_box, n_chunks, tiles_x,
-                               g->gv.sx, g->gv.sy, g->d_tile_cnt, g->d_items, g->d_cursor);
+            hipLaunchKernelGGL(tile_items_wg_kernel, dim3(n_tiles), dim3(1024), 0, st, g->d_chunk_box, g->d_chunk_sector, n_chunks, tiles_x,
+                               g->gv.sx, g->gv.sy, g->d_tile_cnt, g->d_items, g->d_cursor, mark);
             hipLaunchKernelGGL(g->merge ? raycast_tiled_kernel<true> : raycast_tiled_kernel<false>, rgrid, dim3(kTileThreads), 0, st,
                                g->gv, g->d_beams, n, g->d_items, (const int *)nullptr, n_tiles, g->d_cursor, tiles_x, chunk, g->ablate,
                                g->d_tile_cnt, n_chunks);
         } else {
-            hipLaunchKernelGGL((tile_items_kernel<0>), tgrid, dim3(256), 0, st, g->d_chunk_box, n_chunks, tiles_x,
-                               n_tiles, g->gv.sx, g->gv.sy, g->d_tile_cnt, item_off, g->d_items);
+            hipLaunchKernelGGL((tile_items_kernel<0>), tgrid, dim3(256), 0, st, g->d_chunk_box, g->d_chunk_sector, n_chunks, tiles_x,
+                               n_tiles, g->gv.sx, g->gv.sy, g->d_tile_cnt, item_off, g->d_items, mark);
             hipLaunchKernelGGL(tile_scan_kernel, dim3(1), dim3(1024), 0, st, g->d_tile_cnt, n_tiles, item_off, g->d_cursor);
-            hipLaunchKernelGGL((tile_items_kernel<1>), tgrid, dim3(256), 0, st, g->d_chunk_box, n_chunks, tiles_x,
-                               n_tiles, g->gv.sx, g->gv.sy, g->d_tile_cnt, item_off, g->d_items);
+            hipLaunchKernelGGL((tile_items_kernel<1>), tgrid, dim3(256), 0, st, g->d_chunk_box, g->d_chunk_sector, n_chunks, tiles_x,
+                               n_tiles, g->gv.sx, g->gv.sy, g->d_tile_cnt, item_off, g->d_items, mark);
             hipLaunchKernelGGL(g->merge ? raycast_tiled_kernel<true> : raycast_tiled_kernel<false>, rgrid, dim3(kTileThreads), 0, st,
                                g->gv, g->d_beams, n, g->d_items, item_off, n_tiles, g->d_cursor, tiles_x, chunk, g->ablate,
                                g->d_tile_cnt, 0);
         }
     } else {
+        const BoxMark mark = {g->gv.dirty, g->gv.sx, g->gv.sy, g->gv.ox, g->gv.oy};
+        hipLaunchKernelGGL(mark_boxes_kernel, dim3(1), dim3(1024), 0, st, g->d_chunk_box, n_chunks, mark);
         hipLaunchKernelGGL(raycast_global_kernel, dim3((n + 255) / 256), dim3(256), 0, st, g->gv, g->d_beams, n);
     }
     SLAM_HIP(hipGetLastError());
@@ -1114,7 +1239,7 @@
     SLAM_TRY(g->d_num_s.alloc(g->cells * sizeof(double)));
     SLAM_TRY(g->d_occ_s.alloc(g->cells));
     SLAM_TRY(g->d_updates.alloc(kUpdateSlots * sizeof(unsigned long long)));
-    SLAM_TRY(g->d_dirty.alloc(8 * sizeof(int)));
+    SLAM_TRY(g->d_dirty.alloc(16 * sizeof(int)));
     GridView &v = g->gv;
     v.sx = size_x;
     v.sy = size_y;
@@ -1146,7 +1271,7 @@
     SLAM_HIP(hipMemsetAsync(g->d_occ_w, 0xff, g->cells, st));
     SLAM_HIP(hipMemsetAsync(g->d_occ_s, 0xff, g->cells, st));
     SLAM_HIP(hipMemsetAsync(g->d_updates, 0, kUpdateSlots * sizeof(unsigned long long), st));
-    SLAM_HIP(hipMemsetAsync(g->d_dirty, 0x7f, 8 * sizeof(int), st));
+    SLAM_HIP(hipMemsetAsync(g->d_dirty, 0x7f, 16 * sizeof(int), st));
     if (g->d_acc) SLAM_HIP(hipMemsetAsync(g->d_acc, 0, 2 * g->cells * sizeof(int32_t), st));
     g->state_from_inorder = false;
     return SLAM_OK;
@@ -1185,7 +1310,7 @@
         SLAM_HIP(hipGetLastError());
     }
     if (row_hi >= row_lo)
-        hipLaunchKernelGGL(ranges_fold_kernel, dim3(1), dim3(64), 0, st, g->gv.dirty, row_lo, row_hi);
+        hipLaunchKernelGGL(ranges_fold_kernel, dim3(1), dim3(64), 0, st, g->gv.dirty, row_lo, row_hi, g->gv.sx);
     else
         hipLaunchKernelGGL(ranges_retire_kernel, dim3(1), dim3(64), 0, st, g->gv.dirty);
     SLAM_HIP(hipGetLastError());
@@ -1197,7 +1322,7 @@
     SLAM_REQUIRE(g, SLAM_E_INVALID, "null handle");
     if (row_hi < row_lo) return SLAM_OK;
     SLAM_REQUIRE(row_lo >= 0 && row_hi < g->gv.sy, SLAM_E_INVALID, "slam_grid_mark_rows: rows %d..%d outside the grid", row_lo, row_hi);
-    hipLaunchKernelGGL(ranges_set_kernel, dim3(1), dim3(64), 0, as_stream(stream), g->gv.dirty, 2, row_lo, row_hi, g->gv.sy);
+    hipLaunchKernelGGL(ranges_set_kernel, dim3(1), dim3(64), 0, as_stream(stream), g->gv.dirty, 2, row_lo, row_hi, g->gv.sx, g->gv.sy);
     SLAM_HIP(hipGetLastError());
     return SLAM_OK;
 }
@@ -1223,7 +1348,7 @@
 {
     SLAM_REQUIRE(g, SLAM_E_INVALID, "null handle");
     g->prm.min_cluster_points = v;
-    hipLaunchKernelGGL(ranges_set_kernel, dim3(1), dim3(64), 0, nullptr, g->gv.dirty, 1, 0, 0, g->gv.sy);
+    hipLaunchKernelGGL(ranges_set_kernel, dim3(1), dim3(64), 0, nullptr, g->gv.dirty, 1, 0, 0, g->gv.sx, g->gv.sy);
     SLAM_HIP(hipGetLastError());
     return SLAM_OK;
 }
@@ -1269,7 +1394,7 @@
     g->shift_y += dy;
     hipLaunchKernelGGL(roll_clear_kernel, grid2d(g), dim3(256), 0, as_stream(stream), v, dx, dy, g->d_num_s,
                        g->d_occ_s);
-    hipLaunchKernelGGL(ranges_set_kernel, dim3(1), dim3(64), 0, as_stream(stream), g->gv.dirty, 1, 0, 0, v.sy);
+    hipLaunchKernelGGL(ranges_set_kernel, dim3(1), dim3(64), 0, as_stream(stream), g->gv.dirty, 1, 0, 0, v.sx, v.sy);
     SLAM_HIP(hipGetLastError());
     return SLAM_OK;
 }
@@ -1323,7 +1448,7 @@
     const int n_chunks = (n + kChunk - 1) / kChunk;
     hipLaunchKernelGGL(beams_from_rays_kernel, dim3(n_chunks), dim3(kChunk), 0, st, g->gv,
                        reinterpret_cast<const float2 *>(d_origin_xy), reinterpret_cast<const float2 *>(d_end_xy),
-                       n, g->d_beams, g->d_chunk_box);
+                       n, g->d_beams, g->d_chunk_box, g->d_chunk_sector);
     SLAM_HIP(hipGetLastError());
     return walk_beams(g, n, st);
 }
@@ -1359,7 +1484,7 @@
     const int n_chunks = (n + kChunk - 1) / kChunk;
     hipLaunchKernelGGL(beams_from_scans_kernel, dim3(n_chunks), dim3(kChunk), 0, st, g->gv,
                        reinterpret_cast<const double2 *>(d_pts), d_scan_off, n_scans, d_R, d_t, n, g->d_beams,
-                       g->d_chunk_box);
+                       g->d_chunk_box, g->d_chunk_sector);
     SLAM_HIP(hipGetLastError());
     return walk_beams(g, n, st);
 }
@@ -1373,7 +1498,7 @@
     else
         hipLaunchKernelGGL(finalize_rows_kernel, dim3(kRangeBlocks), dim3(256), 0, as_stream(stream), g->gv, g->prm.occupancy_increment,
                            g->prm.occupancy_decrement, (double)g->prm.min_cluster_points, g->d_num_w, g->d_occ_w, g->gv.dirty);
-    hipLaunchKernelGGL(ranges_set_kernel, dim3(1), dim3(64), 0, as_stream(stream), g->gv.dirty, 0, 0, 0, g->gv.sy);
+    hipLaunchKernelGGL(ranges_set_kernel, dim3(1), dim3(64), 0, as_stream(stream), g->gv.dirty, 0, 0, 0, g->gv.sx, g->gv.sy);
     SLAM_HIP(hipGetLastError());
     g->state_from_inorder = false;
     return SLAM_OK;
@@ -1394,7 +1519,7 @@
         SLAM_TRY(slam_grid_finalize(g, stream));
         return slam_grid_reset_counts(g, stream);
     }
-    int *cur = g->gv.dirty, *next = cur == g->d_dirty ? g->d_dirty + 4 : g->d_dirty;
+    int *cur = g->gv.dirty, *next = cur == g->d_dirty ? g->d_dirty + 8 : g->d_dirty;
     hipLaunchKernelGGL(finalize_reset_rows_kernel, dim3(kRangeBlocks), dim3(256), 0, as_stream(stream), g->gv, g->prm.occupancy_increment,
                        g->prm.occupancy_decrement, (double)g->prm.min_cluster_points, g->d_num_w, g->d_occ_w, cur, next);
     SLAM_HIP(hipGetLastError());
```
